# SamsungLabs/Metis

Hardware: NVIDIA H100
Metric: candidate plans evaluated/sec (higher is better)
Workload: dtype f64

## Files before the change

metis_b200/csrc/metis_blob.cuh:

```cuda
#pragma once

#include <cuda_runtime.h>
#include <stdint.h>

#include "metis_eval.cuh"

namespace metis {

struct BlobLayout {
    uint32_t total;
    uint32_t key, lc, mem, exec_full, fb, norm, derived, tmem, bwf, bwm, runt, rune, q10e;
    uint32_t rsum, rsum_bytes;
};

static inline uint32_t align16(uint32_t v) { return (v + 15u) & ~15u; }

static inline BlobLayout make_layout(const MetisProblem &p) {
    BlobLayout l;
    uint32_t o = 0;
    const uint32_t nkey = (uint32_t)p.num_types * p.num_tp * p.num_bs;
    l.key = o;       o = align16(o + nkey * 2);
    l.lc = o;        o = align16(o + (uint32_t)p.num_keys * p.lpad * 8);
    l.mem = o;       o = align16(o + (uint32_t)p.num_keys * p.lpad * 8);
    l.exec_full = o; o = align16(o + (uint32_t)p.num_keys * 8);
    l.fb = o;        o = align16(o + (uint32_t)p.num_keys * 8);
    l.norm = o;      o = align16(o + (uint32_t)p.norm_len * 8);
    l.derived = o;   o = align16(o + (uint32_t)derived_layout(p).total * 8);
    l.tmem = o;      o = align16(o + (uint32_t)p.num_types * 8);
    l.bwf = o;       o = align16(o + (uint32_t)p.num_types * 8);
    l.bwm = o;       o = align16(o + (uint32_t)p.num_types * 8);
    l.runt = o;      o = align16(o + (uint32_t)p.num_node_sequences * p.num_types);
    l.rune = o;      o = align16(o + (uint32_t)p.num_node_sequences * p.num_types * 4);
    l.q10e = o;      o = align16(o + (uint32_t)p.num_node_sequences * p.num_types * 4);
    l.total = o;
    const uint64_t n = (uint64_t)p.num_layers + 1;
    l.rsum = (o + 127u) & ~127u;
    l.rsum_bytes = (uint32_t)((uint64_t)(2 * p.num_keys + 1) * n * n * 8);
    return l;
}

__device__ __forceinline__ Tables make_tables(const MetisProblem &p, const BlobLayout &l, const uint8_t *base,
                                              const uint8_t *gblob = nullptr) {
    Tables T;
    T.p = p;
    T.rsum = gblob ? reinterpret_cast<const double *>(gblob + l.rsum) : nullptr;
    T.key_index = reinterpret_cast<const int16_t *>(base + l.key);
    T.lc = reinterpret_cast<const double *>(base + l.lc);
    T.mem = reinterpret_cast<const double *>(base + l.mem);
    T.exec_full = reinterpret_cast<const double *>(base + l.exec_full);
    T.fb_sync = reinterpret_cast<const double *>(base + l.fb);
    T.norm_lc = reinterpret_cast<const double *>(base + l.norm);
    bind_derived(T, reinterpret_cast<const double *>(base + l.derived));
    T.type_memory = reinterpret_cast<const double *>(base + l.tmem);
    T.bw_first = reinterpret_cast<const double *>(base + l.bwf);
    T.bw_min = reinterpret_cast<const double *>(base + l.bwm);
    T.run_type = base + l.runt;
    T.run_end = reinterpret_cast<const int32_t *>(base + l.rune);
    T.q10_end = reinterpret_cast<const int32_t *>(base + l.q10e);
    return T;
}

__device__ __forceinline__ int find_block(const MetisPlanSpace &sp, int64_t ordinal) {
    int lo = 0, hi = sp.num_blocks - 1;
    while (lo < hi) {
        const int mid = (lo + hi + 1) >> 1;
        if (__ldg(&sp.blocks[mid].first_ordinal) <= ordinal) lo = mid; else hi = mid - 1;
    }
    return lo;
}

__device__ __forceinline__ bool decode_plan(const MetisPlanSpace &sp, int64_t ordinal, PlanDesc &pd, int hint = -1) {
    if (ordinal < 0 || ordinal >= sp.num_plans) return false;
    int lo;
    if (hint >= 0) {
        lo = hint;
        while (lo + 1 < sp.num_blocks && __ldg(&sp.blocks[lo + 1].first_ordinal) <= ordinal) ++lo;
    } else {
        lo = find_block(sp, ordinal);
    }
    const MetisPlanBlock b = sp.blocks[lo];
    const int64_t rel = ordinal - b.first_ordinal;
    const int64_t row = rel / sp.num_div;
    const int div = (int)(rel - row * sp.num_div);
    pd.ordinal = (uint32_t)ordinal;
    pd.ns = b.ns_idx;
    pd.S = b.num_stage;
    pd.label = b.label_stage;
    pd.batches = __ldg(&sp.batches[div]);
    const int64_t off = b.rows_offset + row * b.num_stage;
    pd.row = sp.rows + off;
    pd.geo = pack_geo(off, b.num_stage, b.label_stage, b.ns_idx, div);
    return true;
}

int stage_replay_tables(const MetisProblem *problem, void *workspace, int64_t workspace_bytes, cudaStream_t stream,
                        BlobLayout &lay, const uint8_t *&blob);

}
```

metis_b200/csrc/metis_coop.cuh:

```cuda
#pragma once

#include "metis_eval.cuh"

namespace metis {

struct CoopMail {
    int m;
    int err;
    int flag;
    int aux;
    double val;
    double val2;
    int k;
    int s_top;
    int top_skip;
    int pad2;
};

struct OneLane {
    bool reverse = false;
    MB_HD int lane() const { return 0; }
    MB_HD int width() const { return 1; }
    MB_HD bool leader() const { return true; }
    MB_HD void sync() const {}
    MB_HD bool any(bool p) const { return p; }
    MB_HD unsigned ballot(bool p) const { return p ? 1u : 0u; }
    MB_HD unsigned match_any(int) const { return 1u; }
    MB_HD int first_ge_window(const double *P, int n, int i0, int lo, double t) const {
        for (int k = 0; k < 32 && i0 + k <= n; ++k)
            if (P[i0 + k] >= t) return (k > 0 || i0 <= lo) ? i0 + k : -1;
        return -1;
    }
    MB_HD int first_ge(const double *P, int n, double t) const {
        int lo = 0, hi = n + 1;
        while (lo < hi) { const int mid = (lo + hi) >> 1; if (P[mid] >= t) hi = mid; else lo = mid + 1; }
        return lo;
    }
    MB_HD int bcast_last(int v) const { return v; }
    MB_HD static void assume_shared(const void *) {}
    MB_HD void argmax_first(double &, int &) const {}
    MB_HD void argmin_first(double &, int &) const {}
    MB_HD void imax_first(int &, int &) const {}
    MB_HD void imin_first(int &, int &) const {}
    MB_HD double max_all(double v) const { return v; }
    MB_HD int incl_scan(int v) const { return v; }
    MB_HD int last_lane(int v) const { return v; }
    MB_HD void mark(int) const {}
    MB_HD void note(int) const {}
    MB_HD void gate(int, int) const {}
};

enum CoopGate { kGateRun = 0, kGateBackward = 1, kGateLeftover = 2, kGateVote = 3, kGateAdjust = 4, kGateMemory = 5,
                kGateCost = 6 };

template <class X>
MB_HD int par_index(const X &, int i, int n) { (void)n; return i; }
MB_HD int par_index(const OneLane &x, int i, int n) { return x.reverse ? n - 1 - i : i; }

#define METIS_PAR(x, var, n) \
    for (int var##_i = (x).lane(), var = par_index((x), var##_i, (n)); var##_i < (n); \
         var##_i += (x).width(), var = par_index((x), var##_i, (n)))

struct FillState {
    int k;
    int s_top;
    bool top_skip;
};

template <int MAXS, int MAXL>
MB_HD_NOINLINE FillState seq_forward(const Tables &T, int S, Scratch<MAXS, MAXL> &w) {
    const int L = T.p.num_layers;
    const double *dlay = T.dlay;
    const int N = kH * L;
    const int lim = (N - 1 - kH) > 0 ? (N - 1 - kH) : 0;
    const int last = S - 1;
    FillState st{0, -1, false};
    if (S > 1) {
        int s = 0, j = 0;
        double c = w.capa[0];
        bool done = false;
#pragma unroll 1
        for (int r = 0; r + 1 < L && !done; ++r) {
            const double d = dlay[r];
            const int nsub = (r == L - 2) ? kH - 1 : kH;
            if (nsub == kH && c > 9.0 * d) {
                c -= d; c -= d; c -= d; c -= d; c -= d; c -= d; c -= d;
                j += kH;
                continue;
            }
#pragma unroll
            for (int q = 0; q < kH; ++q) {
                if (q < nsub && !done) {
                    if (c > d) {
                        c -= d;
                    } else {
                        w.capa[s] = c;
                        w.fe[s] = (uint16_t)((j + q) | kBroke);
                        ++s;
                        if (s >= last) done = true;
                        else c = w.capa[s];
                    }
                }
            }
            j += nsub;
        }
        if (s < last) {
            w.capa[s] = c;
            w.fe[s] = (uint16_t)lim;
#pragma unroll 1
            for (int t = s + 1; t < last; ++t) w.fe[t] = (uint16_t)lim;
            st.k = lim;
            st.s_top = s;
        } else {
            st.k = (w.fe[last - 1] & kPos) + 1;
            st.s_top = last - 1;
            st.top_skip = true;
        }
    }
    return st;
}

template <int MAXS, int MAXL>
MB_HD_NOINLINE int seq_backward(const Tables &T, int S, Scratch<MAXS, MAXL> &w, int k) {
    const int L = T.p.num_layers;
    const double *dlay = T.dlay;
    const int N = kH * L;
    const int last = S - 1;
    double c = w.capa[last];
    int r = L - 1;
    double d = dlay[r];
#pragma unroll 1
    for (int i = 0; i < kH; ++i) c -= d;
    int m = N - kH;
    bool full = false;
#pragma unroll 1
    while (m > k && !full) {
        --r;
        d = dlay[r];
        const int floor_j = kH * r > k ? kH * r : k;
#pragma unroll 1
        while (m > floor_j) {
            if (!(c > d)) { full = true; break; }
            c -= d;
            --m;
        }
    }
    if (!full) {
        int sp = S - 2;
#pragma unroll 1
        while (m > 0) {
            const int j = m - 1;
#pragma unroll 1
            while (sp >= 0 && (!(w.fe[sp] & kBroke) || (int)(w.fe[sp] & kPos) > j)) --sp;
            if (!(sp >= 0 && (int)(w.fe[sp] & kPos) == j)) break;
            const double dj = dlay[j / kH];
            if (!(c > dj)) break;
            c -= dj;
            m = j;
            w.fe[sp] |= kTaken;
        }
    }
    w.capa[last] = c;
    return m;
}

template <int MAXS, int MAXL>
MB_HD_NOINLINE int seq_skipped(const Tables &T, int S, Scratch<MAXS, MAXL> &w) {
    const double *dlay = T.dlay;
    const int last = S - 1;
    int start = 0;
#pragma unroll 1
    for (int s = 0; s < last; ++s) {
        const uint16_t e = w.fe[s];
        const int pos = e & kPos;
        const int next_start = pos + ((e & kBroke) ? 1 : 0);
        if ((e & (kBroke | kTaken)) != kBroke) { start = next_start; continue; }
        const int j = pos;
        int lo = 0;
        if (pos > start) {
            lo = s;
        } else {
#pragma unroll 1
            for (int u = s;; --u) {
                if (u < s) {
                    const int t = w.lstk[u];
                    const bool above = (t == last) || (fwd_nonempty(w, t) && fwd_start(w, t) > j);
                    if (!above) { lo = t; break; }
                }
                if (fwd_nonempty(w, u)) { lo = u; break; }
                if (u == 0) break;
            }
        }
        int hi = s + 1;
        if (hi < last && !((int)(w.fe[hi] & kPos) > next_start && !w.got[hi])) {
            ++hi;
#pragma unroll 1
            while (hi < last && (!fwd_nonempty(w, hi) || w.got[hi])) ++hi;
        }
        if (lo > hi) return METIS_FATAL_SCRATCH;
        int pick = lo;
        double best = w.capa[lo];
#pragma unroll 1
        for (int t = lo + 1; t <= hi; ++t)
            if (w.capa[t] > best) { best = w.capa[t]; pick = t; }
        w.capa[pick] -= dlay[j / kH];
        w.lstk[s] = (uint8_t)pick;
        w.got[pick] = 1;
        start = next_start;
    }
    return METIS_FATAL_NONE;
}

template <int MAXS, int MAXL>
MB_HD int middle_lo(int S, const Scratch<MAXS, MAXL> &w, const FillState &st) {
    const int last = S - 1;
    if (st.s_top < 0) return 0;
#pragma unroll 1
    for (int u = st.s_top;; --u) {
        if (u < st.s_top || st.top_skip) {
            const uint16_t eu = w.fe[u];
            if ((eu & (kBroke | kTaken)) == kBroke) {
                const int t2 = w.lstk[u];
                if (t2 != last) return t2;
            }
        }
        if (fwd_nonempty(w, u)) return u;
        if (u == 0) break;
    }
    return 0;
}

MB_HD_NOINLINE double seq_py_sum(const double *v, int n) {
    if (n <= 0) return 0.0;
    double f = 0.0 + v[0], c = 0.0;
#pragma unroll 4
    for (int i = 1; i < n; ++i) {
        const double x = v[i];
        const double t = f + x;
        if (fabs(f) >= fabs(x)) c += (f - t) + x;
        else c += (x - t) + f;
        f = t;
    }
    if (c != 0.0 && isfinite(c)) f += c;
    return f;
}

template <class X>
MB_HD_NOINLINE int psub_search(const X &x, const double *P, int N, int i0, int lo, double t) {
    int i = x.first_ge_window(P, N, i0, lo, t);
    if (i < 0) {
        x.note(kPathFirstGe);
        i = x.first_ge(P, N, t);
        if (i < lo) i = lo;
    }
    return i;
}

MB_HD unsigned bucket_of(double u) {
#ifdef __CUDA_ARCH__
    return __double2uint_rz(u);
#else
    return u > 0.0 ? (unsigned)u : 0u;
#endif
}

template <class X>
MB_HD int psub_lookup(const X &x, const double *P, const uint16_t *IX, double scale, int N, int lo, double t, double &p) {
    int i = IX[bucket_of(t * scale)];
    if (i < lo) i = lo;
    const double *q = P + i;
    const double pm = q[-1], p0 = q[0], p1 = q[1];
    if ((pm < t || i == lo) && p1 >= t) {
        const bool up = !(p0 >= t);
        p = up ? p1 : p0;
        return up ? i + 1 : i;
    }
    i = psub_search(x, P, N, i, lo, t);
    p = P[i];
    return i;
}

template <int MAXS, int MAXL, class X, bool ONE = false>
struct CoopEvaluator : PlanEvaluator<MAXS, MAXL, SerialUniform, ONE> {
    using Base = PlanEvaluator<MAXS, MAXL, SerialUniform, ONE>;
    using Base::T; using Base::w; using Base::pd; using Base::bs_total; using Base::nbad; using Base::aux;
    X x;
    CoopMail &mail;

    MB_HD CoopEvaluator(const Tables &t, Scratch<MAXS, MAXL> &s, CoopMail &mb, const X &lanes)
        : Base(t, s), x(lanes), mail(mb) {}

    MB_HD void shared_scratch() const { X::assume_shared(&w); X::assume_shared(&mail); }

    MB_HD void begin_coop(const PlanDesc &plan) {
        shared_scratch();
        pd = plan;
        bs_total = T.p.gbs / pd.batches;
        int lb = 0;
#pragma unroll 1
        while ((2 << lb) <= bs_total) ++lb;
        nbad = 0;
        x.sync();
        int carry = 0;
#pragma unroll 1
        for (int base = 0; base < pd.S; base += x.width()) {
            const int s = base + x.lane();
            const int g = s < pd.S ? pd.row[s] : 0;
            const int sz = s < pd.S ? (1 << g) : 0;
            const int inc = x.incl_scan(sz);
            if (s < pd.S) {
                w.gcode[s] = (uint8_t)g;
                w.tpc[s] = (uint8_t)(g > lb ? g - lb : 0);
                w.rs[s] = (uint16_t)(carry + inc - sz);
            }
            carry += x.last_lane(inc);
        }
        if (x.leader()) w.rs[pd.S] = (uint16_t)carry;
        x.sync();
    }

    MB_HD bool next_strategy_coop(bool have_state) {
        shared_scratch();
        int pick = 0x7FFFFFFF;
        if (have_state) {
            double best = INFINITY;
            bool none = true;
            METIS_PAR(x, s, pd.S) {
                if (w.gcode[s] != w.tpc[s] && (none || w.mstate[s] < best || (w.mstate[s] == best && s < pick))) {
                    pick = s; best = w.mstate[s]; none = false;
                }
            }
            x.argmin_first(best, pick);
        } else {
            int best = -1;
            METIS_PAR(x, s, pd.S) {
                const int ldp = (int)w.gcode[s] - (int)w.tpc[s];
                if (ldp != 0 && (ldp > best || (ldp == best && s < pick))) { pick = s; best = ldp; }
            }
            x.imax_first(best, pick);
        }
        if (pick == 0x7FFFFFFF) return false;
        const int g = w.gcode[pick], t = w.tpc[pick];
        nbad += (this->stage_bad(g, t + 1) ? 1 : 0) - (this->stage_bad(g, t) ? 1 : 0);
        x.sync();
        if (x.leader()) w.tpc[pick] = (uint8_t)(t + 1);
        x.sync();
        return true;
    }

    MB_HD_NOINLINE int first_error(const double *box, int n) {
        shared_scratch();
        x.sync();
        if (x.leader()) {
            mail.err = 0;
#pragma unroll 1
            for (int s = 0; s < n; ++s)
                if (box[s] != 0.0) {
                    uint32_t a;
                    mail.err = decode_error(box[s], a);
                    mail.aux = (int)a;
                    break;
                }
        }
        x.sync();
        aux = (uint32_t)mail.aux;
        return mail.err;
    }

    MB_HD int compute_performance_coop() {
        shared_scratch();
        bool failed = false;
        x.sync();
        METIS_PAR(x, s, pd.S) {
            double p;
            const int rc = this->stage_performance(s, p);
            w.perf[s] = p;
            w.extra[s] = encode_error(rc, aux);
            failed = failed || rc != 0;
        }
        if (x.any(failed)) return first_error(w.extra, pd.S);
        x.sync();
        if (x.leader()) mail.val = seq_py_sum(w.perf, pd.S);
        x.sync();
        const double tot = mail.val;
        if (tot == 0.0) return METIS_FATAL_ZERODIV;
        METIS_PAR(x, s, pd.S) w.perf[s] = w.perf[s] / tot;
        x.sync();
        return 0;
    }

    MB_HD bool forward_coop() {
        shared_scratch();
        const int S = pd.S, last = S - 1;
        const int L = T.p.num_layers;
        if (S < 4 || T.p.norm_len < L) { x.note(kPathSeqForward); return false; }
        const int N = kH * L;
        const int lim = (N - 1 - kH) > 0 ? (N - 1 - kH) : 0;
        const double *dsub = T.dsub;
        const double *P = T.psub;
        int a = 0, first_open = -1;
        const double scale = T.pidx[0];
        if (scale > 0.0) {
            const uint16_t *IX = reinterpret_cast<const uint16_t *>(T.pidx + 1);
            const double plim = P[lim];
            double pa = P[0];
            int s = 0;
#pragma unroll 1
            for (; s < last; ++s) {
                const double t = w.perf[s] + pa;
                if (!(a < lim && t <= plim)) break;
                const int i = psub_lookup(x, P, IX, scale, N, a + 1, t, pa);
                if (x.leader()) { w.first[s] = (uint16_t)a; w.fe[s] = (uint16_t)((i - 1) | kBroke); }
                a = i;
            }
            if (s < last) {
                first_open = s;
                if (x.leader()) {
#pragma unroll 1
                    for (int u = s; u < last; ++u) { w.first[u] = (uint16_t)(u == s ? a : lim); w.fe[u] = (uint16_t)lim; }
                }
                a = lim;
            }
        } else {
            int span = lim / last;
#pragma unroll 1
            for (int s = 0; s < last; ++s) {
                int b = lim;
                bool closed = false;
                if (a < lim) {
                    const double t = w.perf[s] + P[a];
                    int i0 = a + span - 14;
                    if (i0 < a + 1) i0 = a + 1;
                    int i = x.first_ge_window(P, N, i0, a + 1, t);
                    if (i < 0) { x.note(kPathFirstGe); i = x.first_ge(P, N, t); }
                    b = i - 1 > a ? i - 1 : a;
                    if (b >= lim) b = lim; else closed = true;
                    span = b - a;
                }
                if (x.leader()) { w.first[s] = (uint16_t)a; w.fe[s] = (uint16_t)(b | (closed ? kBroke : 0)); }
                if (!closed && first_open < 0) first_open = s;
                a = closed ? b + 1 : lim;
            }
        }
        x.sync();
        x.mark(19);
        bool bad = false;
        METIS_PAR(x, s, last) {
            const int st = w.first[s];
            const uint16_t e = w.fe[s];
            const int b = e & kPos;
            double c = w.perf[s];
            bool fits = true;
#pragma unroll 4
            for (int j = st; j < b; ++j) {
                const double d = dsub[j];
                fits &= c > d;
                c -= d;
            }
            if (!fits || ((e & kBroke) && c > dsub[b])) bad = true;
            w.capa[s] = c;
        }
        if (x.any(bad)) {
            x.note(kPathVerifyFailed);
            x.sync();
            METIS_PAR(x, s, last) w.capa[s] = w.perf[s];
            return false;
        }
        if (x.leader()) {
            if (first_open < 0) { mail.k = a; mail.s_top = last - 1; mail.top_skip = 1; }
            else { mail.k = lim; mail.s_top = first_open; mail.top_skip = 0; }
        }
        return true;
    }

    MB_HD int fill_coop() {
        shared_scratch();
        const int S = pd.S, last = S - 1;
        const double *dlay = T.dlay;
        x.sync();
        const bool fwd = forward_coop();
        x.sync();
        x.gate(kGateBackward, 11);
        if (x.leader()) {
            if (!fwd) {
                x.mark(18);
                const FillState st = seq_forward<MAXS, MAXL>(T, S, w);
                mail.k = st.k; mail.s_top = st.s_top; mail.top_skip = st.top_skip ? 1 : 0;
                x.mark(11);
            }
            mail.m = seq_backward<MAXS, MAXL>(T, S, w, mail.k);
            mail.err = 0;
        }
        x.sync();
        x.gate(kGateLeftover, 12);
        const FillState st{mail.k, mail.s_top, mail.top_skip != 0};
        const int m = mail.m;
        if (st.s_top >= 0 && !st.top_skip) x.note(kPathTail);
        const int reach = st.s_top;
        bool irregular = false;
        METIS_PAR(x, s, reach + 1) {
            const int start = s == 0 ? 0 : (int)(w.fe[s - 1] & kPos) + ((w.fe[s - 1] & kBroke) ? 1 : 0);
            if (!((int)(w.fe[s] & kPos) > start)) irregular = true;
        }
        irregular = x.any(irregular);
        if (irregular) {
            x.note(kPathIrregular);
            if (x.leader()) mail.err = seq_skipped<MAXS, MAXL>(T, S, w);
            x.sync();
            if (mail.err) return mail.err;
        } else if (reach >= 0) {
            int carry = 0;
#pragma unroll 1
            for (int base = 0; base <= last; base += x.width()) {
                const int s = base + x.lane();
                bool has = false, o0 = false, o1 = false, has_prev = false;
                double c = 0.0, d = 0.0, d_prev = 0.0;
                int pos = 0;
                if (s <= last) {
                    c = w.capa[s];
                    if (s > 0 && s - 1 < last) {
                        const uint16_t ep = w.fe[s - 1];
                        has_prev = (ep & (kBroke | kTaken)) == kBroke;
                        if (has_prev) d_prev = dlay[(ep & kPos) / kH];
                    }
                    if (s < last) {
                        const uint16_t e = w.fe[s];
                        has = (e & (kBroke | kTaken)) == kBroke;
                        if (has) {
                            pos = e & kPos;
                            d = dlay[pos / kH];
                            const double cn = w.capa[s + 1];
                            o0 = cn > c;
                            o1 = has_prev ? cn > (c - d_prev) : o0;
                        }
                    }
                }
                const unsigned kmask = x.ballot(o0 == o1), vmask = x.ballot(o0);
                const unsigned below_me = x.lane() ? (0xFFFFFFFFu >> (32 - x.lane())) : 0u;
                const unsigned kin = kmask & below_me;
                const bool in = kin ? ((vmask >> (31 - clz32(kin))) & 1u) != 0u : carry != 0;
                const bool up = (o0 == o1) ? o0 : in;
                carry = x.bcast_last(up ? 1 : 0);
                x.sync();
                if (s <= last) {
                    double cc = c;
                    const bool got_prev = has_prev && in;
                    if (got_prev) cc -= d_prev;
                    if (has && !up) cc -= d;
                    if (got_prev || (has && !up)) w.capa[s] = cc;
                    if (has) w.lstk[s] = (uint8_t)(up ? s + 1 : s);
                }
            }
            x.sync();
        }
        x.mark(17);
        if (m > st.k) {
            x.note(kPathMiddle);
            if (x.leader()) mail.flag = middle_lo<MAXS, MAXL>(S, w, st);
            x.sync();
            int lo = mail.flag;
#pragma unroll 1
            for (int j = st.k; j < m; ++j) {
                int pick = 0x7FFFFFFF;
                double best = -INFINITY;
#pragma unroll 1
                for (int t = lo + x.lane(); t <= last; t += x.width())
                    if (w.capa[t] > best || (w.capa[t] == best && t < pick)) { best = w.capa[t]; pick = t; }
                x.argmax_first(best, pick);
                x.sync();
                if (x.leader()) {
                    w.capa[pick] = best - dlay[j / kH];
                    reinterpret_cast<uint8_t *>(w.subw)[j - st.k] = (uint8_t)pick;
                }
                x.sync();
                if (pick != last) lo = pick;
            }
        }
        return METIS_FATAL_NONE;
    }

    MB_HD int balance_coop() {
        shared_scratch();
        const int S = pd.S;
        const int L = T.p.num_layers;
        if (T.p.norm_len < L) return METIS_FATAL_INDEX;
        const double *lc = T.norm_lc;
        const int last = S - 1;
        x.sync();
        METIS_PAR(x, s, S) { w.capa[s] = w.perf[s]; w.got[s] = 0; }
        x.sync();
        x.mark(10);
        const int rc_tail = fill_coop();
        if (rc_tail) return rc_tail;
        const int m = mail.m;
        x.gate(kGateVote, 13);
        const int kfwd = mail.k;
        const int B = (L + 31) >> 5;
        METIS_PAR(x, blk, 32) {
            const int r0 = blk * B, r1 = r0 + B < L ? r0 + B : L;
            const int j0 = kH * r0;
            int t = 0;
            if (j0 < kfwd && j0 < m) {
                int lo = 0, hi = last - 1;
#pragma unroll 1
                while (lo < hi) {
                    const int mid = (lo + hi) >> 1;
                    const uint16_t e = w.fe[mid];
                    if ((int)(e & kPos) + ((e & kBroke) ? 1 : 0) <= j0) lo = mid + 1; else hi = mid;
                }
                t = lo;
            }
            uint16_t e = w.fe[t];
            int nxt = (int)(e & kPos) + ((e & kBroke) ? 1 : 0);
#pragma unroll 1
            for (int r = r0; r < r1; ++r) {
                int own = last;
                if (kH * r < m) {
                    uint64_t v = 0xFF00000000000000ULL;
#pragma unroll 1
                    for (int q = 0; q < kH; ++q) {
                        const int j = kH * r + q;
                        int st;
                        if (j >= m) st = last;
                        else if (j >= kfwd) st = reinterpret_cast<const uint8_t *>(w.subw)[j - kfwd];
                        else {
#pragma unroll 1
                            while (nxt <= j) { ++t; e = w.fe[t]; nxt = (int)(e & kPos) + ((e & kBroke) ? 1 : 0); }
                            st = t;
                            if (nxt - 1 == j && (e & kBroke)) st = (e & kTaken) ? last : (int)w.lstk[t];
                        }
                        v |= (uint64_t)st << (8 * q);
                    }
                    own = layer_owner(v, (T.p.corrected & METIS_FIX_Q5) != 0);
                }
                reinterpret_cast<uint8_t *>(w.ownerw)[r] = (uint8_t)own;
            }
        }
        METIS_PAR(x, s, S) w.cnt[s] = 0;
        x.sync();
        x.mark(14);
#pragma unroll 1
        for (int base = 0; base < L; base += x.width()) {
            const int r = base + x.lane();
            const int own = r < L ? (int)reinterpret_cast<const uint8_t *>(w.ownerw)[r] : (int)kDropped;
            const unsigned peers = x.match_any(own);
            if (own != (int)kDropped && x.lane() == ctz32(peers)) {
                const int n = popc32(peers), lo_r = r, hi_r = base + 31 - clz32(peers);
                const int have = w.cnt[own];
                if (have == 0 || lo_r < (int)w.first[own]) w.first[own] = (uint16_t)lo_r;
                if (have == 0 || hi_r > (int)w.lastl[own]) w.lastl[own] = (uint16_t)hi_r;
                w.cnt[own] = (uint16_t)(have + n);
            }
            x.sync();
        }
        METIS_PAR(x, s, S) {
            const int n = w.cnt[s];
            w.capa[s] = n ? w.perf[s] - range_sum<SerialUniform>(T, kRangeNorm, 0, lc, w.first[s], (int)w.lastl[s] + 1) : w.perf[s];
        }
        x.sync();
        x.gate(kGateAdjust, 15);
        uint8_t *owner = reinterpret_cast<uint8_t *>(w.ownerw);
#pragma unroll 1
        for (int n = 1; n <= 3; ++n) {
            int top = 0x7FFFFFFF;
            double maxc = -INFINITY;
            METIS_PAR(x, t, S)
                if (w.capa[t] > maxc || (w.capa[t] == maxc && t < top)) { maxc = w.capa[t]; top = t; }
            x.argmax_first(maxc, top);
            if (top == 0x7FFFFFFF) top = 0;
            int nb = -1;
            double val = INFINITY;
            if (top - 1 >= 0 && w.capa[top - 1] < val) { nb = top - 1; val = w.capa[top - 1]; }
            if (top + 1 < S && w.capa[top + 1] < val) { nb = top + 1; }
            if (nb < 0 || w.cnt[nb] <= 1) break;
            const int layer = (top > nb) ? w.lastl[nb] : w.first[nb];
            const double dl = lc[layer];
            const double ntop = w.capa[top] - dl;
            const double nnb = w.capa[nb] + dl;
            double newmax = -INFINITY;
            METIS_PAR(x, t, S) {
                const double v = (t == top) ? ntop : (t == nb) ? nnb : w.capa[t];
                if (v > newmax) newmax = v;
            }
            newmax = x.max_all(newmax);
            if (newmax > maxc) break;
            x.sync();
            if (x.leader()) {
                owner[layer] = (uint8_t)top;
                w.capa[top] = ntop;
                w.capa[nb] = nnb;
                if (top > nb) { int r = layer - 1; while (owner[r] != nb) --r; w.lastl[nb] = (uint16_t)r; }
                else          { int r = layer + 1; while (owner[r] != nb) ++r; w.first[nb] = (uint16_t)r; }
                if (w.cnt[top] == 0) { w.first[top] = (uint16_t)layer; w.lastl[top] = (uint16_t)layer; }
                else {
                    if (layer < (int)w.first[top]) w.first[top] = (uint16_t)layer;
                    if (layer > (int)w.lastl[top]) w.lastl[top] = (uint16_t)layer;
                }
                ++w.cnt[top];
                --w.cnt[nb];
            }
            x.sync();
        }
        x.mark(16);
        int carry = 0;
#pragma unroll 1
        for (int base = 0; base < S; base += x.width()) {
            const int s = base + x.lane();
            const int v = s < S ? (int)w.cnt[s] : 0;
            const int inc = x.incl_scan(v);
            if (s < S) w.part[s + 1] = (uint16_t)(carry + inc);
            carry += x.last_lane(inc);
        }
        if (x.leader()) w.part[0] = 0;
        x.sync();
        return METIS_FATAL_NONE;
    }

    MB_HD int adjust_performance_coop() {
        shared_scratch();
        const int S = pd.S;
        double *ratio = reinterpret_cast<double *>(w.subw);
        x.sync();
        METIS_PAR(x, s, S) {
            double av, adj, extra;
            this->stage_adjust(s, av, adj, extra);
            w.capa[s] = av;
            w.mstate[s] = adj;
            ratio[s] = extra;
        }
        x.sync();
        if (x.leader()) {
            double need = 0.;
#pragma unroll 4
            for (int s = 0; s < S; ++s) need += ratio[s];
            mail.val = need;
            mail.flag = seq_py_sum(w.capa, S) < need ? 1 : 0;
        }
        x.sync();
        if (mail.flag) return 1;
        METIS_PAR(x, s, S) w.extra[s] = 0.;
        x.sync();
        if (x.leader()) {
            double need = mail.val;
            int guard = 0;
            mail.err = 0;
#pragma unroll 1
            while (need > 0.01) {
                PySum tot;
#pragma unroll 4
                for (int s = 0; s < S; ++s) tot.add(w.capa[s] > 0.001 ? w.perf[s] : 0.0);
                const double tmp_total = tot.result();
#pragma unroll 4
                for (int s = 0; s < S; ++s)
                    ratio[s] = w.capa[s] > 0.001 ? w.perf[s] / tmp_total : 0.0;
#pragma unroll 4
                for (int s = 0; s < S; ++s) {
                    const double av = w.capa[s];
                    const double want = need * ratio[s];
                    const double give = want > av ? av : want;
                    w.extra[s] += give;
                    w.capa[s] -= give;
                    need -= give;
                }
                if (++guard > 4096) { mail.err = METIS_FATAL_HANG; break; }
            }
        }
        x.sync();
        if (mail.err) return -mail.err;
        METIS_PAR(x, s, S) w.perf[s] = w.extra[s] + w.mstate[s];
        x.sync();
        return 0;
    }

    template <class Sink>
    MB_HD int memory_phase_coop(int attempt, Sink &sink, bool report) {
        shared_scratch();
        const int S = pd.S;
        bool failed = false, oom = false;
        x.sync();
        METIS_PAR(x, s, S) {
            double md, state;
            const int rc = this->stage_memory(s, md, state);
            w.extra[s] = md;
            w.capa[s] = state;
            w.mstate[s] = encode_error(rc, aux);
            failed = failed || rc != 0;
            oom = oom || state < 0;
        }
        failed = x.any(failed);
        oom = x.any(oom);
        if (failed) return -first_error(w.mstate, S);
        x.sync();
        if (!oom) {
            METIS_PAR(x, s, S) w.mstate[s] = w.capa[s];
            x.sync();
            return 1;
        }
        if constexpr (SinkMisses<Sink>::value) {
            if (report) {
                double m = INFINITY;
                int at = 0x7FFFFFFF;
                METIS_PAR(x, s, S)
                    if (w.capa[s] < m || (w.capa[s] == m && s < at)) { m = w.capa[s]; at = s; }
                x.argmin_first(m, at);
                sink.miss(pd, attempt, -m, at);
            }
        } else {
            (void)sink, (void)report;
        }
        if (attempt >= 3) return 0;
        x.mark(21);
        const int rc = adjust_performance_coop();
        if (rc < 0) return rc;
        return rc == 1 ? 0 : 2;
    }

    MB_HD int get_cost_coop(double &cost_out) {
        shared_scratch();
        const bool one_type = ONE || T.p.num_types == 1;
        const int nstage = pd.label < pd.S ? pd.label : pd.S;
        if (T.p.q10_devices < T.p.total_devices && this->rank_start(nstage) > T.p.q10_devices) return 1;
        double *ppterm = reinterpret_cast<double *>(w.subw);
        bool bad = false;
        double max_len = -INFINITY, max_upd = -INFINITY, max_dp = -INFINITY;
        x.sync();
        METIS_PAR(x, s, nstage) {
            double len, dpc, upd;
            if (this->stage_time(s, len)) bad = true;
            w.capa[s] = len;
            if (len > max_len) max_len = len;
            this->stage_terms(s, nstage, ppterm[s], dpc, upd);
            if (dpc > max_dp) max_dp = dpc;
            if (upd > max_upd) max_upd = upd;
        }
        if (x.any(bad)) return 1;
        max_len = x.max_all(max_len);
        max_upd = x.max_all(max_upd);
        max_dp = x.max_all(max_dp);
        x.sync();
        x.mark(23);
        if (x.leader()) {
            double pp_cost = 0.;
#pragma unroll 4
            for (int s = 0; s + 1 < nstage; ++s) pp_cost += ppterm[s];
            const double lens = seq_py_sum(w.capa, nstage);
            const int s = nstage - 1;
            const int a = one_type ? 0 : this->rank_start(s), b = a + this->group(s);
            double v = 0.0;
            mail.flag = this->fb_sync_cost(a, b, w.tpc[s], bs_total >> (w.gcode[s] - w.tpc[s]), v);
            const double fb_sync = v * (double)pd.batches;
            const double exec = ((double)(pd.batches - 1) * max_len) + lens;
            const double bg = T.p.batch_generator * (double)pd.batches;
            mail.val = exec + fb_sync + max_upd + max_dp + pp_cost + bg;
        }
        x.sync();
        if (mail.flag) return 1;
        cost_out = mail.val;
        return 0;
    }

    enum Start { kFresh = 0, kReplay = 1, kRetry = 2, kAdvance = 3 };
    template <class Sink>
    MB_HD void run_chain(const PlanDesc &plan, Sink &sink, int start, const double *perf = nullptr, size_t perf_stride = 0) {
        begin_coop(plan);
        bool started = false, have_state = false;
        bool skip_first = start == kReplay;
        int nrep = 0, step = 0;
        int call = start == kAdvance ? 1 : 0;
        if (start == kRetry) {
            METIS_PAR(x, s, pd.S) w.perf[s] = perf[(size_t)s * perf_stride];
            x.sync();
        }
#pragma unroll 1
        for (;;) {
            if (nrep == 1) return;
            int attempt = 0;
#pragma unroll 1
            for (;;) {
                int first_attempt = 1;
                if (!started) {
                    started = true;
                    if (start == kAdvance && !next_strategy_coop(false)) return;
                    if (start == kRetry) first_attempt = 2;
                } else if (!next_strategy_coop(have_state)) return;
                if (!this->valid()) continue;
                miss_call(sink, call++);
                int rc = 0;
                if (first_attempt == 1) {
                    if (!skip_first) sink.partition_call();
                    x.mark(2);
                    rc = compute_performance_coop();
                    if (rc) { sink.fatal(pd.ordinal, rc, aux); return; }
                }
                attempt = 0;
#pragma unroll 1
                for (int a = first_attempt; a <= 3; ++a) {
                    const bool fresh = !skip_first;
                    if (fresh) sink.balancer_run();
                    skip_first = false;
                    x.gate(kGateRun, 9);
                    rc = balance_coop();
                    if (rc) { sink.fatal(pd.ordinal, rc, aux); return; }
                    x.gate(kGateMemory, 20);
                    const int r = memory_phase_coop(a, sink, fresh);
                    if (r < 0) { sink.fatal(pd.ordinal, -r, aux); return; }
                    if (r == 1) { attempt = a; break; }
                    if (r == 0) break;
                }
                skip_first = false;
                have_state = attempt > 0;
                if (attempt > 0) break;
            }
            nrep = attempt;
            x.gate(kGateCost, 22);
            double cost = 0.0;
            if (get_cost_coop(cost) == 0) sink.emit(pd, step, nrep, cost, w.tpc, w.part);
            else sink.keyerror();
            x.sync();
            x.mark(24);
            ++step;
        }
    }
};

}
```

metis_b200/csrc/metis_eval.cuh:

```cuda
#pragma once

#include <stdint.h>
#include <string.h>
#include <math.h>

#include "../../include/metis_b200.h"

#if defined(__CUDACC__)
#define MB_HD __host__ __device__ __forceinline__
#define MB_HD_NOINLINE __host__ __device__ __noinline__ inline
#else
#define MB_HD inline
#define MB_HD_NOINLINE inline
#endif

namespace metis {

constexpr int kH = 7;
constexpr double kMemCoef = 5.0;
constexpr uint8_t kDropped = 0xFF;

struct Tables {
    MetisProblem p;
    const int16_t *key_index;
    const double *lc;
    const double *mem;
    const double *exec_full;
    const double *fb_sync;
    const double *norm_lc;
    const double *type_memory, *bw_first, *bw_min;
    const uint8_t *run_type;
    const int32_t *run_end;
    const int32_t *q10_end;
    const double *dlay;
    const double *inv_exec;
    const double *ratio;
    const double *dpk;
    const double *pp_hidden;
    const double *pp_vocab;
    const double *psub;
    const double *dsub;
    const double *pidx;
    const double *rsum;
};

constexpr int kDpk = 16;

struct DerivedLayout {
    int dlay, inv_exec, ratio, dpk, pp_hidden, pp_vocab, psub, dsub, pidx, total;
};

MB_HD DerivedLayout derived_layout(const MetisProblem &p) {
    DerivedLayout d;
    int o = 0;
    d.dlay = o; o += p.norm_len;
    d.inv_exec = o; o += p.num_keys;
    d.ratio = o; o += p.num_layers + 1;
    d.dpk = o; o += kDpk;
    d.pp_hidden = o; o += p.num_bs + 1;
    d.pp_vocab = o; o += (p.num_bs + 1) * p.num_tp;
    d.psub = o; o += (p.norm_len >= p.num_layers) ? kH * p.num_layers + 1 : 0;
    d.dsub = o; o += (p.norm_len >= p.num_layers) ? kH * p.num_layers : 0;
    d.pidx = o; o += (p.norm_len >= p.num_layers) ? 1 + (kH * p.num_layers + 1 + 3) / 4 : 0;
    d.total = o;
    return d;
}

MB_HD double psub_at(double acc, double lc_r, int q) { return acc + lc_r * ((double)q / 7.0); }

MB_HD double psub_index_entry(const MetisProblem &p, const double *norm_lc, int k) {
    const int L = p.num_layers, N = kH * L;
    const int lim = (N - 1 - kH) > 0 ? (N - 1 - kH) : 0;
    bool ok = N > 0;
    double acc = 0.0;
    for (int r = 0; r < L; ++r) {
        ok = ok && norm_lc[r] >= 0.0 && norm_lc[r] <= 1.7976931348623157e308;
        acc += norm_lc[r];
    }
    const double top = L < p.norm_len ? psub_at(acc, norm_lc[L], 0) : acc;
    const double scale = ok && top > 0.0 && top <= 1.7976931348623157e308 ? (double)N / top : 0.0;
    if (!(scale > 0.0 && scale <= 1.7976931348623157e308)) return 0.0;
    if (k == 0) return scale;
    double f[kH];
    for (int q = 0; q < kH; ++q) f[q] = (double)q / 7.0;
    uint64_t bits = 0;
    int r = 0;
    acc = 0.0;
    for (int e = 0; e < 4; ++e) {
        const double g = (double)(4 * (k - 1) + e);
        int ix = lim;
        while (kH * r < lim) {
            const double nxt = acc + norm_lc[r];
            if (nxt * scale >= g) {
                int q = 0;
                while (q < kH && !((acc + norm_lc[r] * f[q]) * scale >= g)) ++q;
                ix = kH * r + q < lim ? kH * r + q : lim;
                break;
            }
            acc = nxt;
            ++r;
        }
        bits |= (uint64_t)ix << (16 * e);
    }
    double v;
    memcpy(&v, &bits, sizeof(v));
    return v;
}

MB_HD double derive_entry(const MetisProblem &p, const DerivedLayout &d, const double *norm_lc,
                          const double *exec_full, const double *bw_first, int i) {
    if (i < d.inv_exec) return norm_lc[i - d.dlay] / 7.0;
    if (i < d.ratio) return 1. / exec_full[i - d.inv_exec];
    if (i < d.dpk) return (double)(i - d.ratio) / (double)p.num_layers;
    const double bw = bw_first[0] * 1048576.0;
    if (i < d.pp_hidden) {
        const int dp = 1 << (i - d.dpk);
        return (double)(2 * (dp - 1)) / ((double)dp * bw);
    }
    if (i < d.pp_vocab) return (double)((int64_t)(i - d.pp_hidden) * p.sequence_length * p.hidden_size) / bw;
    if (i >= d.pidx) return psub_index_entry(p, norm_lc, i - d.pidx);
    if (i >= d.dsub) return norm_lc[(i - d.dsub) / kH] / 7.0;
    if (i >= d.psub) {
        const int j = i - d.psub, r = j / kH;
        double acc = 0.0;
        for (int t = 0; t < r; ++t) acc += norm_lc[t];
        return r < p.norm_len ? psub_at(acc, norm_lc[r], j - r * kH) : acc;
    }
    const int e = i - d.pp_vocab;
    const int mbs = e / p.num_tp, tpc = e - mbs * p.num_tp;
    return ((double)((int64_t)mbs * p.sequence_length * p.vocab_size) / (double)(1 << tpc)) / bw;
}

MB_HD void bind_derived(Tables &T, const double *base) {
    const DerivedLayout d = derived_layout(T.p);
    T.dlay = base + d.dlay;
    T.inv_exec = base + d.inv_exec;
    T.ratio = base + d.ratio;
    T.dpk = base + d.dpk;
    T.pp_hidden = base + d.pp_hidden;
    T.pp_vocab = base + d.pp_vocab;
    T.psub = base + d.psub;
    T.dsub = base + d.dsub;
    T.pidx = base + d.pidx;
}

struct PlanDesc {
    uint32_t ordinal;
    int ns;
    int S;
    int label;
    int batches;
    const uint8_t *row;
    uint64_t geo;
};

MB_HD uint64_t pack_geo(int64_t row_offset, int S, int label, int ns, int div) {
    return (uint64_t)(row_offset & 0xFFFFFFFFLL) | ((uint64_t)((S - 1) & 0xFF) << 32) | ((uint64_t)((label - 1) & 0xFF) << 40) |
           ((uint64_t)(ns & 0xFF) << 48) | ((uint64_t)(div & 0xFF) << 56);
}

enum BalancerPath {
    kPathVerifyFailed = 0,
    kPathSeqForward = 1,
    kPathIrregular = 2,
    kPathMiddle = 3,
    kPathFirstGe = 4,
    kPathTail = 5,
    kPathVoteEnds = 6,
};

struct Serial {
    static constexpr bool kUniform = false;
    MB_HD void mark(int) const {}
    MB_HD void note(int) const {}
    MB_HD void converge() const {}
    MB_HD void rejoin(bool) {}
};
#if defined(__CUDACC__) && defined(METIS_PROFILE_PHASES)
constexpr int kBulkBatches = 31;
__device__ long long g_bulk_acc[32];
__shared__ long long s_bulk_t[32];
__shared__ int s_bulk_cur[32];
__device__ __forceinline__ void bulk_mark(unsigned group, int id) {
    __syncwarp(group);
    if ((int)(threadIdx.x & 31) == __ffs((int)group) - 1) {
        const int wi = threadIdx.x >> 5;
        const long long now = clock64();
        if (id == 1) atomicAdd((unsigned long long *)&g_bulk_acc[kBulkBatches], 1ULL);
        else atomicAdd((unsigned long long *)&g_bulk_acc[s_bulk_cur[wi] & 31], (unsigned long long)(now - s_bulk_t[wi]));
        s_bulk_cur[wi] = id;
        s_bulk_t[wi] = now;
    }
    __syncwarp(group);
}
#endif
#if defined(__CUDACC__)
struct Lockstep : Serial {
    unsigned mask;
    __device__ Lockstep() : mask(0xFFFFFFFFu) {}
    __device__ void converge() const { __syncwarp(mask); }
    __device__ void rejoin(bool p) { mask = __ballot_sync(0xFFFFFFFFu, p); }
#if defined(METIS_PROFILE_PHASES)
    __device__ void mark(int id) const { bulk_mark(__activemask(), id); }
#endif
};
#endif
struct SerialUniform : Serial {
    static constexpr bool kUniform = true;
};

constexpr uint64_t kOnes = 0x0101010101010101ULL;

constexpr uint16_t kBroke = 0x8000;
constexpr uint16_t kTaken = 0x4000;
constexpr uint16_t kPos = 0x3FFF;

template <int MAXS, int MAXL>
struct Scratch {
    double perf[MAXS];
    double capa[MAXS];
    double mstate[MAXS];
    double extra[MAXS];
    uint16_t fe[MAXS];
    uint16_t first[MAXS], lastl[MAXS], cnt[MAXS];
    uint16_t part[MAXS + 1];
    uint16_t rs[MAXS + 1];
    uint8_t gcode[MAXS];
    uint8_t tpc[MAXS];
    uint8_t lstk[MAXS];
    uint8_t got[MAXS];
    uint64_t ownerw[MAXL / 8 + 1];
    uint64_t subw[MAXL];
    static_assert(MAXL >= MAXS, "after the vote, subw holds one double per stage (CoopEvaluator's adjust and cost)");
};

MB_HD double py_sum_range(const double *x, int a, int b) {
    if (a >= b) return 0.0;
    double f = 0.0 + x[a];
    double c = 0.0;
    for (int i = a + 1; i < b; ++i) {
        const double v = x[i];
        const double t = f + v;
        if (fabs(f) >= fabs(v)) c += (f - t) + v;
        else c += (v - t) + f;
        f = t;
    }
    if (c != 0.0 && isfinite(c)) f += c;
    return f;
}

MB_HD_NOINLINE double py_sum_range_compact(const double *x, int a, int b) {
    if (a >= b) return 0.0;
    double f = 0.0 + x[a];
    double c = 0.0;
#pragma unroll 1
    for (int i = a + 1; i < b; ++i) {
        const double v = x[i];
        const double t = f + v;
        if (fabs(f) >= fabs(v)) c += (f - t) + v;
        else c += (v - t) + f;
        f = t;
    }
    if (c != 0.0 && isfinite(c)) f += c;
    return f;
}

template <class X>
MB_HD double sum_range(const double *x, int a, int b) {
    if constexpr (X::kUniform) return py_sum_range_compact(x, a, b);
    else return py_sum_range(x, a, b);
}

MB_HD void fill_range_sums(const double *row, int L, int a, double *out) {
    const int n = L + 1;
    double f = 0.0 + row[a];
    double c = 0.0;
    out[(size_t)(a + 1) * n + a] = f;
#if defined(__CUDA_ARCH__)
#pragma unroll 1
#endif
    for (int i = a + 1; i < L; ++i) {
        const double v = row[i];
        const double t = f + v;
        if (fabs(f) >= fabs(v)) c += (f - t) + v;
        else c += (v - t) + f;
        f = t;
        out[(size_t)(i + 1) * n + a] = (c != 0.0 && isfinite(c)) ? f + c : f;
    }
}
MB_HD int range_sum_tables(const MetisProblem &p) { return 2 * p.num_keys + 1; }
MB_HD const double *range_sum_row(const MetisProblem &p, int t, const double *mem, const double *lc, const double *norm) {
    if (t < p.num_keys) return mem + (size_t)t * p.lpad;
    if (t < 2 * p.num_keys) return lc + (size_t)(t - p.num_keys) * p.lpad;
    return p.norm_len >= p.num_layers ? norm : nullptr;
}

enum RangeTable { kRangeMem = 0, kRangeLc = 1, kRangeNorm = 2 };
template <class X>
MB_HD double range_sum(const Tables &T, int family, int key, const double *row, int a, int b) {
    if (a >= b) return 0.0;
    if (T.rsum && b <= T.p.num_layers) {
        const int n = T.p.num_layers + 1;
        const int t = family == kRangeMem ? key : family == kRangeLc ? T.p.num_keys + key : 2 * T.p.num_keys;
#if defined(__CUDA_ARCH__)
        return __ldg(&T.rsum[((size_t)t * n + b) * n + a]);
#else
        return T.rsum[((size_t)t * n + b) * n + a];
#endif
    }
    return sum_range<X>(row, a, b);
}

struct PySum {
    double f, c;
    int n;
    MB_HD PySum() : f(0.0), c(0.0), n(0) {}
    MB_HD void add(double v) {
        if (n == 0) { f = 0.0 + v; }
        else {
            const double t = f + v;
            if (fabs(f) >= fabs(v)) c += (f - t) + v;
            else c += (v - t) + f;
            f = t;
        }
        ++n;
    }
    MB_HD double result() const {
        double r = f;
        if (c != 0.0 && isfinite(c)) r += c;
        return r;
    }
};

MB_HD double pow2_neg(int k) {
    const uint64_t bits = (uint64_t)(1023 - k) << 52;
    double d;
    memcpy(&d, &bits, sizeof(d));
    return d;
}

MB_HD int type_of_rank(const Tables &T, int ns, int rank) {
    const int nt = T.p.num_types;
    const int32_t *end = T.run_end + ns * nt;
    const uint8_t *typ = T.run_type + ns * nt;
#pragma unroll 1
    for (int k = 0; k < nt; ++k)
        if (rank < end[k]) return typ[k];
    return typ[nt - 1];
}

MB_HD int type_of_q10(const Tables &T, int ns, int idx) {
    const int nt = T.p.num_types;
    const int32_t *end = T.q10_end + ns * nt;
    const uint8_t *typ = T.run_type + ns * nt;
#pragma unroll 1
    for (int k = 0; k < nt; ++k)
        if (idx < end[k]) return typ[k];
    return typ[nt - 1];
}

MB_HD int key_of(const Tables &T, int type, int tpc, int bs) {
    if (tpc >= T.p.num_tp || bs < 1 || bs > T.p.num_bs) return -1;
    return T.key_index[(type * T.p.num_tp + tpc) * T.p.num_bs + (bs - 1)];
}

template <int MAXS, int MAXL>
MB_HD int fwd_start(const Scratch<MAXS, MAXL> &w, int s) {
    if (s == 0) return 0;
    const uint16_t e = w.fe[s - 1];
    return (e & kPos) + ((e & kBroke) ? 1 : 0);
}

template <int MAXS, int MAXL>
MB_HD bool fwd_nonempty(const Scratch<MAXS, MAXL> &w, int s) {
    return (int)(w.fe[s] & kPos) > fwd_start(w, s);
}

MB_HD int popc64(uint64_t v) {
#if defined(__CUDA_ARCH__)
    return __popcll(v);
#else
    return __builtin_popcountll(v);
#endif
}
MB_HD int ctz64(uint64_t v) {
#if defined(__CUDA_ARCH__)
    return __ffsll((long long)v) - 1;
#else
    return __builtin_ctzll(v);
#endif
}
MB_HD int popc32(uint32_t v) {
#if defined(__CUDA_ARCH__)
    return __popc(v);
#else
    return __builtin_popcount(v);
#endif
}
MB_HD int ctz32(uint32_t v) {
#if defined(__CUDA_ARCH__)
    return __ffs((int)v) - 1;
#else
    return __builtin_ctz(v);
#endif
}
MB_HD int clz32(uint32_t v) {
#if defined(__CUDA_ARCH__)
    return __clz((int)v);
#else
    return __builtin_clz(v);
#endif
}
MB_HD int clz64(uint64_t v) {
#if defined(__CUDA_ARCH__)
    return __clzll((long long)v);
#else
    return __builtin_clzll(v);
#endif
}

MB_HD uint64_t swar_eq(uint64_t x, int c) {
    const uint64_t y = x ^ ((uint64_t)c * kOnes);
    const uint64_t lo7 = 0x7F7F7F7F7F7F7F7FULL;
    return ~((((y & lo7) + lo7) | y) | lo7);
}

MB_HD int swar_count(uint64_t x, int c) { return popc64(swar_eq(x, c) & 0x0080808080808080ULL); }

MB_HD int layer_owner(uint64_t v, bool plurality) {
    if (plurality) {
        int best = 0, own = (int)kDropped;
#pragma unroll 1
        for (int q = 0; q < kH; ++q) {
            const int cq = (int)((v >> (8 * q)) & 0xFF);
            const int n = swar_count(v, cq);
            if (n > best || (n == best && cq < own)) { best = n; own = cq; }
        }
        return own;
    }
    const int c3 = (int)((v >> 24) & 0xFF);
    if (swar_count(v, c3) * 2 > kH) return c3;
    const int c0 = (int)(v & 0xFF), c1 = (int)((v >> 8) & 0xFF), c2 = (int)((v >> 16) & 0xFF);
    if (swar_count(v, c0) * 2 > kH) return c0;
    if (c1 != c0 && swar_count(v, c1) * 2 > kH) return c1;
    if (c2 != c1 && c2 != c0 && swar_count(v, c2) * 2 > kH) return c2;
    return (int)kDropped;
}

template <int MAXS, int MAXL, class X>
MB_HD int balance_run(const Tables &T, int S, Scratch<MAXS, MAXL> &w, const X &x) {
    const int L = T.p.num_layers;
    if (T.p.norm_len < L) return METIS_FATAL_INDEX;
    const double *dlay = T.dlay;
    const double *lc = T.norm_lc;
    const int N = kH * L;
    const int lim = (N - 1 - kH) > 0 ? (N - 1 - kH) : 0;
    const int last = S - 1;
    int broken = METIS_FATAL_NONE;

#pragma unroll (X::kUniform ? 1 : 0)
    for (int s = 0; s < S; ++s) { w.got[s] = 0; w.cnt[s] = 0; }

    x.mark(10);
    int k = 0, sTop = -1;
    bool topSkip = false;
    if (S > 1) {
        int s = 0, j = 0;
        double c = w.perf[0];
#pragma unroll (X::kUniform ? 1 : 0)
        for (int r = 0; r + 1 < L; ++r) {
            const double d = dlay[r];
            const int nsub = (r == L - 2) ? kH - 1 : kH;
#pragma unroll
            for (int q = 0; q < kH; ++q) {
                if (q < nsub) {
                    if (s < last) {
                        if (c > d) {
                            c -= d;
                        } else {
                            w.capa[s] = c;
                            w.fe[s] = (uint16_t)(j | kBroke);
                            ++s;
                            c = w.perf[s];
                        }
                    }
                    ++j;
                }
            }
        }
        if (s < last) {
            x.note(kPathTail);
            w.capa[s] = c;
            w.fe[s] = (uint16_t)lim;
#pragma unroll (X::kUniform ? 1 : 0)
            for (int t = s + 1; t < last; ++t) { w.capa[t] = w.perf[t]; w.fe[t] = (uint16_t)lim; }
            k = lim;
            sTop = s;
        } else {
            k = (w.fe[last - 1] & kPos) + 1;
            sTop = last - 1;
            topSkip = true;
        }
    }

    x.mark(11);
    x.converge();
    int m;
    {
        double c = w.perf[last];
        const double dl = dlay[L - 1];
#pragma unroll (X::kUniform ? 1 : 0)
        for (int i = 0; i < kH; ++i) c -= dl;
        m = N - kH;
        int sp = S - 2;
#pragma unroll (X::kUniform ? 1 : 0)
        while (m > 0) {
            const int j = m - 1;
            bool un = (j >= k);
            if (!un) {
#pragma unroll (X::kUniform ? 1 : 0)
                while (sp >= 0 && (!(w.fe[sp] & kBroke) || (int)(w.fe[sp] & kPos) > j)) --sp;
                un = (sp >= 0 && (int)(w.fe[sp] & kPos) == j);
            }
            if (!un) break;
            const double d = dlay[j / kH];
            if (!(c > d)) break;
            c -= d;
            m = j;
            if (j < k) w.fe[sp] |= kTaken;
        }
        w.capa[last] = c;
    }

    x.mark(12);
    x.converge();
    {
        int start = 0;
#pragma unroll (X::kUniform ? 1 : 0)
        for (int s = 0; s < last; ++s) {
            const uint16_t e = w.fe[s];
            const int pos = e & kPos;
            const int next_start = pos + ((e & kBroke) ? 1 : 0);
            if ((e & (kBroke | kTaken)) != kBroke) { start = next_start; continue; }
            const int j = pos;
            int lo = 0;
            if (pos > start) {
                lo = s;
            } else {
                x.note(kPathIrregular);
#pragma unroll (X::kUniform ? 1 : 0)
                for (int u = s;; --u) {
                    if (u < s) {
                        const int t = w.lstk[u];
                        const bool above = (t == last) || (fwd_nonempty(w, t) && fwd_start(w, t) > j);
                        if (!above) { lo = t; break; }
                    }
                    if (fwd_nonempty(w, u)) { lo = u; break; }
                    if (u == 0) break;
                }
            }
            int hi = s + 1;
            if (hi < last && !((int)(w.fe[hi] & kPos) > next_start && !w.got[hi])) {
                ++hi;
#pragma unroll (X::kUniform ? 1 : 0)
                while (hi < last && (!fwd_nonempty(w, hi) || w.got[hi])) ++hi;
            }
            if (lo > hi) { broken = METIS_FATAL_SCRATCH; hi = lo; }
            int pick = lo;
            double best = w.capa[lo];
#pragma unroll (X::kUniform ? 1 : 0)
            for (int t = lo + 1; t <= hi; ++t)
                if (w.capa[t] > best) { best = w.capa[t]; pick = t; }
            w.capa[pick] -= dlay[j / kH];
            w.lstk[s] = (uint8_t)pick;
            w.got[pick] = 1;
            start = next_start;
        }
    }
    x.converge();
    const int nblk = m - k;
    if (nblk > 0) x.note(kPathMiddle);
    uint8_t *mid = reinterpret_cast<uint8_t *>(w.subw);
    {
        int below = -1;
#pragma unroll (X::kUniform ? 1 : 0)
        for (int t = 0; t < nblk; ++t) {
            const int j = k + t;
            int lo = 0;
            if (below >= 0) lo = below;
            else if (sTop >= 0) {
#pragma unroll (X::kUniform ? 1 : 0)
                for (int u = sTop;; --u) {
                    if (u < sTop || topSkip) {
                        const uint16_t eu = w.fe[u];
                        if ((eu & (kBroke | kTaken)) == kBroke) {
                            const int t2 = w.lstk[u];
                            if (t2 != last) { lo = t2; break; }
                        }
                    }
                    if (fwd_nonempty(w, u)) { lo = u; break; }
                    if (u == 0) break;
                }
            }
            int pick = lo;
            double best = w.capa[lo];
#pragma unroll (X::kUniform ? 1 : 0)
            for (int t2 = lo + 1; t2 <= last; ++t2)
                if (w.capa[t2] > best) { best = w.capa[t2]; pick = t2; }
            w.capa[pick] -= dlay[j / kH];
            if (pick != last) below = pick;
            mid[t] = (uint8_t)pick;
        }
    }

    x.mark(13);
    x.converge();
    if (k > 0) x.note(kPathVoteEnds);
    int t = 0, nxt = 0;
    uint16_t e = 0;
    if (k > 0) { e = w.fe[0]; nxt = (int)(e & kPos) + ((e & kBroke) ? 1 : 0); }
    const bool plurality = (T.p.corrected & METIS_FIX_Q5) != 0;
    int run_own = (int)kDropped, run_first = 0, run_len = 0;
#pragma unroll (X::kUniform ? 1 : 0)
    for (int r = 0; r < L; ++r) {
        int own = last;
        if (kH * r < m) {
            uint64_t v = 0xFF00000000000000ULL;
#pragma unroll
            for (int q = 0; q < kH; ++q) {
                const int j = kH * r + q;
                int st = last;
                if (j < k) {
#pragma unroll 1
                    while (nxt <= j) { ++t; e = w.fe[t]; nxt = (int)(e & kPos) + ((e & kBroke) ? 1 : 0); }
                    st = t;
                    if (nxt - 1 == j && (e & kBroke)) st = (e & kTaken) ? last : (int)w.lstk[t];
                } else if (j < m) {
                    st = mid[j - k];
                }
                v |= (uint64_t)(uint32_t)st << (8 * q);
            }
            own = layer_owner(v, plurality);
        }
        reinterpret_cast<uint8_t *>(w.ownerw)[r] = (uint8_t)own;
        {
            if (own == run_own) ++run_len;
            else {
                if (run_own != (int)kDropped) {
                    if (w.cnt[run_own] == 0) w.first[run_own] = (uint16_t)run_first;
                    w.lastl[run_own] = (uint16_t)(r - 1);
                    w.cnt[run_own] = (uint16_t)(w.cnt[run_own] + run_len);
                }
                run_own = own; run_first = r; run_len = 1;
            }
        }
    }
    if (run_own != (int)kDropped) {
        if (w.cnt[run_own] == 0) w.first[run_own] = (uint16_t)run_first;
        w.lastl[run_own] = (uint16_t)(L - 1);
        w.cnt[run_own] = (uint16_t)(w.cnt[run_own] + run_len);
    }
    x.mark(14);
    x.converge();
    uint8_t *owner = reinterpret_cast<uint8_t *>(w.ownerw);
    int top = 0x7FFFFFFF;
    double maxc = -INFINITY;
#pragma unroll (X::kUniform ? 1 : 0)
    for (int s = 0; s < S; ++s) {
        const double c = w.cnt[s] ? w.perf[s] - range_sum<X>(T, kRangeNorm, 0, lc, w.first[s], (int)w.lastl[s] + 1) : w.perf[s];
        w.capa[s] = c;
        if (c > maxc) { maxc = c; top = s; }
    }

    x.mark(15);
    x.converge();
#pragma unroll (X::kUniform ? 1 : 0)
    for (int n = 1; n <= 3; ++n) {
        if (top == 0x7FFFFFFF) top = 0;
        int nb = -1;
        double val = INFINITY;
        if (top - 1 >= 0 && w.capa[top - 1] < val) { nb = top - 1; val = w.capa[top - 1]; }
        if (top + 1 < S && w.capa[top + 1] < val) { nb = top + 1; }
        if (nb < 0 || w.cnt[nb] <= 1) break;
        const int layer = (top > nb) ? w.lastl[nb] : w.first[nb];
        const double dl = lc[layer];
        const double ntop = w.capa[top] - dl;
        const double nnb = w.capa[nb] + dl;
        double newmax = -INFINITY;
        int newtop = 0x7FFFFFFF;
#pragma unroll (X::kUniform ? 1 : 0)
        for (int t = 0; t < S; ++t) {
            const double v = (t == top) ? ntop : (t == nb) ? nnb : w.capa[t];
            if (v > newmax) { newmax = v; newtop = t; }
        }
        if (newmax > maxc) break;
        owner[layer] = (uint8_t)top;
        w.capa[top] = ntop;
        w.capa[nb] = nnb;
        if (top > nb) { int r = layer - 1; while (owner[r] != nb) --r; w.lastl[nb] = (uint16_t)r; }
        else          { int r = layer + 1; while (owner[r] != nb) ++r; w.first[nb] = (uint16_t)r; }
        if (w.cnt[top] == 0) { w.first[top] = (uint16_t)layer; w.lastl[top] = (uint16_t)layer; }
        else {
            if (layer < (int)w.first[top]) w.first[top] = (uint16_t)layer;
            if (layer > (int)w.lastl[top]) w.lastl[top] = (uint16_t)layer;
        }
        ++w.cnt[top];
        --w.cnt[nb];
        maxc = newmax;
        top = newtop;
    }

    x.mark(16);
    x.converge();
    w.part[0] = 0;
#pragma unroll (X::kUniform ? 1 : 0)
    for (int s = 0; s < S; ++s) w.part[s + 1] = (uint16_t)(w.part[s] + w.cnt[s]);
    return broken;
}

struct HSplit {
    int nruns;
    int type[METIS_MAX_TYPES];
    int n[METIS_MAX_TYPES];
    int base[METIS_MAX_TYPES];
    int plus[METIS_MAX_TYPES];
};

MB_HD_NOINLINE int partition_data(const Tables &T, int ns, int rank_lo, int count, int dp, int tpc, int bs,
                                  HSplit &out, uint32_t &aux, bool q10 = false) {
    const int gsz = count / dp;
    double perf[METIS_MAX_TYPES];
    PySum total;
    out.nruns = 0;
#pragma unroll 1
    for (int i = 0; i < dp; ++i) {
        const int t = q10 ? type_of_q10(T, ns, rank_lo + i * gsz) : type_of_rank(T, ns, rank_lo + i * gsz);
        if (out.nruns == 0 || out.type[out.nruns - 1] != t) {
            const int key = key_of(T, t, tpc, 1);
            if (key < 0) { aux = ((uint32_t)tpc << 16) | 1u; return METIS_FATAL_KEY_EXEC; }
            const double e = T.exec_full[key];
            if (e == 0.0) return METIS_FATAL_ZERODIV;
            out.type[out.nruns] = t;
            out.n[out.nruns] = 0;
            perf[out.nruns] = 1. / e;
            ++out.nruns;
        }
        ++out.n[out.nruns - 1];
        total.add(perf[out.nruns - 1]);
    }
    const double tot = total.result();
    double frac[METIS_MAX_TYPES];
    int assigned = 0;
#pragma unroll 1
    for (int r = 0; r < out.nruns; ++r) {
        const double v = (double)bs * (perf[r] / tot);
        const int b = (int)v;
        out.base[r] = b;
        out.plus[r] = 0;
        frac[r] = v - (double)b;
        assigned += b * out.n[r];
    }
    int rem = bs - assigned;
    bool used[METIS_MAX_TYPES];
#pragma unroll 1
    for (int r = 0; r < out.nruns; ++r) used[r] = false;
#pragma unroll 1
    for (int it = 0; it < out.nruns && rem > 0; ++it) {
        int pick = -1;
#pragma unroll 1
        for (int r = 0; r < out.nruns; ++r)
            if (!used[r] && (pick < 0 || frac[r] > frac[pick])) pick = r;
        used[pick] = true;
        const int g = rem < out.n[pick] ? rem : out.n[pick];
        out.plus[pick] = g;
        rem -= g;
    }
    if (rem > 0) return METIS_FATAL_SCRATCH;
    return METIS_FATAL_NONE;
}

template <class Sink, class = void>
struct SinkMisses { static constexpr bool value = false; };
template <class Sink>
struct SinkMisses<Sink, decltype(void(Sink::kMisses))> { static constexpr bool value = Sink::kMisses; };
template <class Sink>
MB_HD void miss_call(Sink &sink, int call) {
    if constexpr (SinkMisses<Sink>::value) sink.call = call;
    else (void)sink, (void)call;
}

struct TraceTap {
    double *demand;
    double *state;
    double cost[5];
};

MB_HD int halvings_of(const MetisProblem &p, int S, const uint8_t *gcode, const uint8_t *tpc, int bs_total) {
    int ltp = 0, lbs = 0;
    while ((2 << ltp) <= p.max_tp) ++ltp;
    while ((2 << lbs) <= p.max_bs) ++lbs;
    int u = 0;
#if defined(__CUDA_ARCH__)
#pragma unroll 1
#endif
    for (int s = 0; s < S; ++s) {
        const int g = gcode[s], t = tpc[s];
        int lm = 0;
        while ((2 << lm) <= (bs_total >> (g - t))) ++lm;
        int room = g - t;
        if (ltp - t < room) room = ltp - t;
        if (lbs - lm < room) room = lbs - lm;
        if (room > 0) u += room;
    }
    return u;
}

MB_HD double encode_error(int rc, uint32_t aux) { return rc ? (double)rc + (double)aux * 256.0 : 0.0; }
MB_HD int decode_error(double word, uint32_t &aux) {
    const uint64_t code = (uint64_t)word;
    aux = (uint32_t)(code >> 8);
    return (int)(code & 0xFF);
}

template <int MAXS, int MAXL, class X = Serial, bool ONE = false>
struct PlanEvaluator {
    const Tables &T;
    Scratch<MAXS, MAXL> &w;
    X x;
    PlanDesc pd;
    int bs_total;
    int nbad;
    uint32_t aux;
    TraceTap *tap;

    MB_HD PlanEvaluator(const Tables &t, Scratch<MAXS, MAXL> &s, const X &lanes = X())
        : T(t), w(s), x(lanes), bs_total(0), nbad(0), aux(0), tap(nullptr) {}

    MB_HD int group(int s) const { return 1 << w.gcode[s]; }
    MB_HD int dp_of(int s) const { return (1 << w.gcode[s]) >> w.tpc[s]; }

    MB_HD bool stage_bad(int g, int t) const {
        const int mbs = bs_total >> (g - t);
        return mbs == 0 || mbs > T.p.max_bs || (1 << t) > T.p.max_tp;
    }

    MB_HD int begin(const PlanDesc &plan) {
        pd = plan;
        if (pd.S > MAXS || T.p.num_layers > MAXL) return -1;
        bs_total = T.p.gbs / pd.batches;
        int lb = 0;
#pragma unroll (X::kUniform ? 1 : 0)
        while ((2 << lb) <= bs_total) ++lb;
        nbad = 0;
        int a = 0;
        for (int s = 0; s < pd.S; ++s) {
            const int g = pd.row[s];
            const int t = g > lb ? g - lb : 0;
            if (stage_bad(g, t)) { nbad = 1; return 0; }
            w.gcode[s] = (uint8_t)g;
            w.rs[s] = (uint16_t)a;
            a += 1 << g;
            w.tpc[s] = (uint8_t)t;
        }
        w.rs[pd.S] = (uint16_t)a;
        return nbad == 0 ? 1 : 0;
    }

    MB_HD bool next_strategy(bool have_state) {
        int pick = -1;
        if (have_state) {
            double best = 0.0;
#pragma unroll (X::kUniform ? 1 : 0)
            for (int s = 0; s < pd.S; ++s)
                if (w.gcode[s] != w.tpc[s] && (pick < 0 || w.mstate[s] < best)) { pick = s; best = w.mstate[s]; }
        } else {
            int best = -1;
#pragma unroll (X::kUniform ? 1 : 0)
            for (int s = 0; s < pd.S; ++s) {
                const int ldp = (int)w.gcode[s] - (int)w.tpc[s];
                if (ldp != 0 && ldp > best) { pick = s; best = ldp; }
            }
        }
        if (pick < 0) return false;
        const int g = w.gcode[pick], t = w.tpc[pick];
        nbad += (stage_bad(g, t + 1) ? 1 : 0) - (stage_bad(g, t) ? 1 : 0);
        w.tpc[pick] = (uint8_t)(t + 1);
        return true;
    }

    MB_HD bool valid() const { return nbad == 0; }

    MB_HD int halvings() const { return halvings_of(T.p, pd.S, w.gcode, w.tpc, bs_total); }

    MB_HD double memory_capacity(int a, int b) const {
        const int nt = T.p.num_types;
        if (ONE || nt == 1) return T.type_memory[0] * (double)(b - a);
        const int32_t *end = T.run_end + pd.ns * nt;
        const uint8_t *typ = T.run_type + pd.ns * nt;
        PySum acc;
        int lo = 0;
#pragma unroll (X::kUniform ? 1 : 0)
        for (int k = 0; k < nt; ++k) {
            const int hi = end[k];
            const int x = (a > lo ? a : lo), y = (b < hi ? b : hi);
            if (y > x) acc.add(T.type_memory[typ[k]] * (double)(y - x));
            lo = hi;
        }
        return acc.result();
    }

    MB_HD int replica_perf_cost(int type, int tpc, int h, double &out) {
        double acc = 0.;
#pragma unroll (X::kUniform ? 1 : 0)
        for (int bit = 30; bit >= 0; --bit) {
            const int piece = 1 << bit;
            if (!(h & piece)) continue;
            const int key = key_of(T, type, tpc, piece);
            if (key < 0) { aux = ((uint32_t)tpc << 16) | (uint32_t)piece; return METIS_FATAL_KEY_EXEC; }
            acc += T.exec_full[key];
        }
        out = acc;
        return 0;
    }

    MB_HD_NOINLINE int hetero_performance(int a, int b, int dp, int tpc, double &p) {
        HSplit hs;
        int rc = partition_data(T, pd.ns, a, b - a, dp, tpc, bs_total, hs, aux);
        if (rc) return rc;
        double mx = -INFINITY;
#pragma unroll (X::kUniform ? 1 : 0)
        for (int r = 0; r < hs.nruns; ++r) {
            double c;
            if (hs.plus[r] > 0) {
                rc = replica_perf_cost(hs.type[r], tpc, hs.base[r] + 1, c);
                if (rc) return rc;
                if (c > mx) mx = c;
            }
            if (hs.plus[r] < hs.n[r]) {
                rc = replica_perf_cost(hs.type[r], tpc, hs.base[r], c);
                if (rc) return rc;
                if (c > mx) mx = c;
            }
        }
        p = (mx != 0.0) ? 1. / mx : 0.0;
        return 0;
    }

    MB_HD int rank_start(int s) const { return w.rs[s]; }


    MB_HD int stage_performance(int s, double &p) {
        const int g = w.gcode[s], tpc = w.tpc[s];
        const int a = rank_start(s), b = a + (1 << g);
        int ta = 0, tb = 0;
        if (!(ONE || T.p.num_types == 1)) { ta = type_of_rank(T, pd.ns, a); tb = type_of_rank(T, pd.ns, b - 1); }
        p = 0.0;
        if (ta != tb) return hetero_performance(a, b, 1 << (g - tpc), tpc, p);
        const int bs = bs_total >> (g - tpc);
        const int key = key_of(T, ta, tpc, bs);
        if (key < 0) { aux = ((uint32_t)tpc << 16) | (uint32_t)bs; return METIS_FATAL_KEY_EXEC; }
        if (T.exec_full[key] == 0.0) return METIS_FATAL_ZERODIV;
        p = T.inv_exec[key];
        return 0;
    }

    MB_HD int stage_memory(int s, double &demand, double &state) {
        const bool one_type = ONE || T.p.num_types == 1;
        const bool own_type = (T.p.corrected & METIS_FIX_Q6) != 0;
        const int g = w.gcode[s], tpc = w.tpc[s];
        const int a = rank_start(s), b = a + (1 << g);
        int rc = 0;
        demand = 0.001;
        if (!ONE && own_type) {
            rc = memory_demand_own_type(s, demand);
        } else if (T.p.q10_devices < T.p.total_devices && !own_type && b > T.p.q10_devices) {
            aux = 0;
            rc = METIS_FATAL_INDEX;
        } else if (one_type || type_of_q10(T, pd.ns, a) == type_of_q10(T, pd.ns, b - 1)) {
            const int bs = bs_total >> (g - tpc);
            const int key = key_of(T, T.run_type[pd.ns * T.p.num_types], tpc, bs);
            if (key < 0) { aux = ((uint32_t)tpc << 16) | (uint32_t)bs; rc = METIS_FATAL_KEY_MEMORY; }
            else demand += range_sum<X>(T, kRangeMem, key, T.mem + (size_t)key * T.p.lpad, w.part[s], w.part[s + 1]) * kMemCoef;
        } else {
            rc = hetero_memory_demand(s, T.run_type[pd.ns * T.p.num_types], demand);
        }
        state = memory_capacity(a, b) - demand;
        return rc;
    }

    MB_HD void stage_adjust(int s, double &avail, double &adj, double &extra) const {
        const double c = w.perf[s], md = w.extra[s];
        const double mc = memory_capacity(rank_start(s), rank_start(s) + group(s));
        if (mc > md) {
            adj = c;
            avail = (c * mc / md) - c;
            extra = 0.0;
        } else {
            avail = 0.0;
            adj = c * (mc / md) * 0.9;
            extra = c - adj;
        }
    }

    MB_HD bool stage_time(int s, double &len) {
        const bool one_type = ONE || T.p.num_types == 1;
        const int g = w.gcode[s], tpc = w.tpc[s];
        const int a = one_type ? 0 : rank_start(s), b = a + (1 << g);
        const int la = w.part[s], lb = w.part[s + 1];
        const int ldp = g - tpc;
        const int ta = one_type ? 0 : type_of_rank(T, pd.ns, a);
        const int tb = one_type ? 0 : type_of_rank(T, pd.ns, b - 1);
        len = 0.0;
        if (ta != tb) return hetero_exec_cost(a, b, 1 << ldp, tpc, la, lb, len) != 0;
        const int key = key_of(T, ta, tpc, bs_total >> ldp);
        if (key < 0) return true;
        len = range_sum<X>(T, kRangeLc, key, T.lc + (size_t)key * T.p.lpad, la, lb);
        return false;
    }

    MB_HD void stage_terms(int s, int nstage, double &pp, double &dpc, double &upd) const {
        const int per = T.p.devices_per_node;
        const int Lm = T.p.num_layers;
        const bool ubw = T.p.uniform_bw != 0;
        const int g = w.gcode[s], tpc = w.tpc[s];
        const int la = w.part[s], lb = w.part[s + 1];
        const int ldp = g - tpc;
        const int mbs = bs_total >> ldp;
        const double inv_tp = pow2_neg(tpc);
        pp = 0.0;
        if (s < nstage - 1) {
            if (ubw) {
                pp = (lb == Lm - 1) ? T.pp_vocab[mbs * T.p.num_tp + tpc] : T.pp_hidden[mbs];
            } else {
                double act;
                if (lb == Lm - 1)
                    act = (double)((int64_t)mbs * T.p.sequence_length * T.p.vocab_size) * inv_tp;
                else
                    act = (double)((int64_t)mbs * T.p.sequence_length * T.p.hidden_size);
                pp = act / (bw_of_node_range(rank_start(s) / per, (rank_start(s + 2) - 1) / per) * 1048576.0);
            }
        }
        int ntr = lb - la;
        double params = 0.0;
        if (la == 0) { params += T.p.input_params * inv_tp; --ntr; }
        if (lb == Lm) { params += T.p.output_params * inv_tp; --ntr; }
        params += T.p.transformer_params * inv_tp * (double)ntr;
        if (ubw) dpc = T.dpk[ldp] * params;
        else {
            const int dp = 1 << ldp;
            dpc = (double)(2 * (dp - 1)) / ((double)dp * (dp_bandwidth(rank_start(s), dp, 1 << tpc) * 1048576.0)) * params;
        }
        upd = T.p.optimizer_time * inv_tp * T.ratio[lb - la];
    }


    MB_HD int compute_performance() {
        PySum total;
        int rc = 0;
#pragma unroll (X::kUniform ? 1 : 0)
        for (int s = 0; s < pd.S; ++s) {
            double p;
            rc = stage_performance(s, p);
            if (rc) break;
            w.perf[s] = p;
            total.add(p);
        }
        x.converge();
        if (rc) return rc;
        const double tot = total.result();
        if (tot == 0.0) return METIS_FATAL_ZERODIV;
#pragma unroll (X::kUniform ? 1 : 0)
        for (int s = 0; s < pd.S; ++s) w.perf[s] = w.perf[s] / tot;
        return 0;
    }

    MB_HD_NOINLINE int hetero_memory_demand(int s, int type0, double &demand) {
        const int la = w.part[s], lb = w.part[s + 1], tpc = w.tpc[s];
        HSplit hs;
        const int rc = partition_data(T, pd.ns, 0, T.p.q10_devices, dp_of(s), tpc, bs_total, hs, aux, true);
        if (rc) return rc;
#pragma unroll (X::kUniform ? 1 : 0)
        for (int r = 0; r < hs.nruns; ++r)
#pragma unroll (X::kUniform ? 1 : 0)
            for (int i = 0; i < hs.n[r]; ++i) {
                const int h = hs.base[r] + (i < hs.plus[r] ? 1 : 0);
#pragma unroll (X::kUniform ? 1 : 0)
                for (int bit = 30; bit >= 0; --bit) {
                    const int piece = 1 << bit;
                    if (!(h & piece)) continue;
                    const int key = key_of(T, type0, tpc, piece);
                    if (key < 0) { aux = ((uint32_t)tpc << 16) | (uint32_t)piece; return METIS_FATAL_KEY_MEMORY; }
                    demand += range_sum<X>(T, kRangeMem, key, T.mem + (size_t)key * T.p.lpad, la, lb) * kMemCoef;
                }
            }
        return 0;
    }

    MB_HD_NOINLINE int memory_demand_own_type(int s, double &demand) {
        const int la = w.part[s], lb = w.part[s + 1], tpc = w.tpc[s], g = w.gcode[s];
        const int a = rank_start(s), b = a + (1 << g);
        const int ta = type_of_rank(T, pd.ns, a), tb = type_of_rank(T, pd.ns, b - 1);
        if (ta == tb) {
            const int bs = bs_total >> (g - tpc);
            const int key = key_of(T, ta, tpc, bs);
            if (key < 0) { aux = ((uint32_t)tpc << 16) | (uint32_t)bs; return METIS_FATAL_KEY_MEMORY; }
            demand += range_sum<SerialUniform>(T, kRangeMem, key, T.mem + (size_t)key * T.p.lpad, la, lb) * kMemCoef;
            return 0;
        }
        HSplit hs;
        const int rc = partition_data(T, pd.ns, a, b - a, 1 << (g - tpc), tpc, bs_total, hs, aux);
        if (rc) return rc;
        double worst = 0.0;
#pragma unroll 1
        for (int r = 0; r < hs.nruns; ++r)
#pragma unroll 1
            for (int v = 0; v < 2; ++v) {
                const int cntv = v ? hs.plus[r] : hs.n[r] - hs.plus[r];
                const int h = hs.base[r] + v;
                if (cntv <= 0 || h == 0) continue;
                double need = 0.0;
#pragma unroll 1
                for (int bit = 30; bit >= 0; --bit) {
                    const int piece = 1 << bit;
                    if (!(h & piece)) continue;
                    const int key = key_of(T, hs.type[r], tpc, piece);
                    if (key < 0) { aux = ((uint32_t)tpc << 16) | (uint32_t)piece; return METIS_FATAL_KEY_MEMORY; }
                    need += range_sum<SerialUniform>(T, kRangeMem, key, T.mem + (size_t)key * T.p.lpad, la, lb) * kMemCoef;
                }
                if (need > worst) worst = need;
            }
        demand += worst;
        return 0;
    }

    MB_HD_NOINLINE int adjust_performance() {
        const int S = pd.S;
        double need = 0.;
        PySum avail_sum;
#pragma unroll (X::kUniform ? 1 : 0)
        for (int s = 0; s < S; ++s) {
            double av, adj, extra;
            stage_adjust(s, av, adj, extra);
            w.capa[s] = av;
            w.mstate[s] = adj;
            w.extra[s] = 0.;
            need += extra;
            avail_sum.add(av);
        }
        if (avail_sum.result() < need) return 1;
        int guard = 0;
#pragma unroll (X::kUniform ? 1 : 0)
        while (need > 0.01) {
            PySum tot;
#pragma unroll (X::kUniform ? 1 : 0)
            for (int s = 0; s < S; ++s) tot.add(w.capa[s] > 0.001 ? w.perf[s] : 0.0);
            const double tmp_total = tot.result();
#pragma unroll (X::kUniform ? 1 : 0)
            for (int s = 0; s < S; ++s) {
                const double av = w.capa[s];
                const double ratio = av > 0.001 ? w.perf[s] / tmp_total : 0.0;
                const double want = need * ratio;
                const double give = want > av ? av : want;
                w.extra[s] += give;
                w.capa[s] -= give;
                need -= give;
            }
            if (++guard > 4096) return -METIS_FATAL_HANG;
        }
#pragma unroll (X::kUniform ? 1 : 0)
        for (int s = 0; s < S; ++s) w.perf[s] = w.extra[s] + w.mstate[s];
        return 0;
    }

    struct NoMisses {};
    MB_HD int memory_phase(int attempt) {
        NoMisses none;
        return memory_phase(attempt, none);
    }
    template <class Sink>
    MB_HD int memory_phase(int attempt, Sink &sink) {
        const int S = pd.S;
        bool oom = false;
        int rc = 0;
#pragma unroll (X::kUniform ? 1 : 0)
        for (int s = 0; s < S; ++s) {
            double md, state;
            rc = stage_memory(s, md, state);
            if (rc) break;
            w.extra[s] = md;
            w.mstate[s] = state;
            if (state < 0) oom = true;
            if (tap) { tap->demand[s] = md; tap->state[s] = state; }
        }
        x.converge();
        if (rc) return -rc;
        if (!oom) return 1;
        if constexpr (SinkMisses<Sink>::value) {
            double m = w.mstate[0];
            int at = 0;
#pragma unroll 1
            for (int s = 1; s < S; ++s)
                if (w.mstate[s] < m) { m = w.mstate[s]; at = s; }
            sink.miss(pd, attempt, -m, at);
        } else {
            (void)sink;
        }
        if (attempt >= 3) return 0;
        x.mark(21);
        const int adj = adjust_performance();
        if (adj < 0) return adj;
        return adj == 1 ? 0 : 2;
    }

    template <class Sink>
    MB_HD_NOINLINE int partition_layer(Sink &sink) {
#pragma unroll (X::kUniform ? 1 : 0)
        for (int attempt = 1; attempt <= 3; ++attempt) {
            sink.balancer_run();
            const int rc = balance_run<MAXS, MAXL>(T, pd.S, w, x);
            if (rc) return -rc;
            const int r = memory_phase(attempt, sink);
            if (r == 1) return attempt;
            if (r <= 0) return r;
        }
        return 0;
    }

    MB_HD double bw_of_node_range(int n0, int n1) const {
        const int per = T.p.devices_per_node;
        if (n0 == n1) return T.bw_first[type_of_q10(T, pd.ns, n0 * per)];
        double slow = INFINITY;
        const int nt = T.p.num_types;
        const int32_t *end = T.q10_end + pd.ns * nt;
        const uint8_t *typ = T.run_type + pd.ns * nt;
        int lo = 0;
#pragma unroll (X::kUniform ? 1 : 0)
        for (int k = 0; k < nt; ++k) {
            const int hi = end[k];
            if (hi > lo && n0 * per < hi && (n1 + 1) * per > lo) {
                const double v = T.bw_min[typ[k]];
                if (v < slow) slow = v;
            }
            lo = hi;
        }
        return slow;
    }

    MB_HD double dp_bandwidth(int a, int dp, int tp) const {
        const int per = T.p.devices_per_node;
        double slow = INFINITY;
#pragma unroll (X::kUniform ? 1 : 0)
        for (int d = 0; d < dp; ++d) {
            const int n0 = (a + d) / per;
            int nlast = n0;
            bool multi = false;
            double gmin = INFINITY;
            int tprev = -1;
#pragma unroll (X::kUniform ? 1 : 0)
            for (int i = 0; i < tp; ++i) {
                const int node = (a + d + i * dp) / per;
                if (node != nlast) { multi = true; nlast = node; }
                const int t = type_of_q10(T, pd.ns, node * per);
                if (t != tprev) { const double v = T.bw_min[t]; if (v < gmin) gmin = v; tprev = t; }
            }
            const double bw = multi ? gmin : T.bw_first[type_of_q10(T, pd.ns, n0 * per)];
            if (bw < slow) slow = bw;
        }
        return slow;
    }

    MB_HD_NOINLINE int hetero_exec_cost(int a, int b, int dp, int tpc, int la, int lb, double &len) {
        HSplit hs;
        uint32_t dummy;
        if (partition_data(T, pd.ns, a, b - a, dp, tpc, bs_total, hs, dummy)) return 1;
        len = -INFINITY;
#pragma unroll (X::kUniform ? 1 : 0)
        for (int r = 0; r < hs.nruns; ++r)
#pragma unroll (X::kUniform ? 1 : 0)
            for (int v = 0; v < 2; ++v) {
                const int cntv = v ? hs.plus[r] : hs.n[r] - hs.plus[r];
                const int h = hs.base[r] + v;
                if (cntv <= 0 || h == 0) continue;
                double acc = 0.;
#pragma unroll (X::kUniform ? 1 : 0)
                for (int bit = 30; bit >= 0; --bit) {
                    const int piece = 1 << bit;
                    if (!(h & piece)) continue;
                    if (piece > T.p.max_bs) return 1;
                    const int key = key_of(T, hs.type[r], tpc, piece);
                    if (key < 0) return 1;
                    acc += range_sum<X>(T, kRangeLc, key, T.lc + (size_t)key * T.p.lpad, la, lb);
                }
                if (acc > len) len = acc;
            }
        return 0;
    }

    MB_HD int fb_sync_cost(int a, int b, int tpc, int mbs, double &out) const {
        const int nt = T.p.num_types;
        const int32_t *end = T.run_end + pd.ns * nt;
        const uint8_t *typ = T.run_type + pd.ns * nt;
        double mx = -INFINITY;
        int lo = 0;
#pragma unroll (X::kUniform ? 1 : 0)
        for (int k = 0; k < nt; ++k) {
            const int hi = end[k];
            if ((a > lo ? a : lo) < (b < hi ? b : hi)) {
                const int key = key_of(T, typ[k], tpc, mbs);
                if (key < 0) return 1;
                const double v = T.fb_sync[key];
                if (v == 0.0) return 1;
                if (v > mx) mx = v;
            }
            lo = hi;
        }
        out = mx;
        return 0;
    }

    MB_HD int get_cost(double &cost_out) {
        const bool one_type = ONE || T.p.num_types == 1;
        const int nstage = pd.label < pd.S ? pd.label : pd.S;
        if (T.p.q10_devices < T.p.total_devices && rank_start(nstage) > T.p.q10_devices) return 1;
        bool bad = false;
        PySum lens_sum;
        double max_len = -INFINITY;
#pragma unroll (X::kUniform ? 1 : 0)
        for (int s = 0; s < nstage; ++s) {
            double len;
            if (stage_time(s, len)) bad = true;
            lens_sum.add(len);
            if (len > max_len) max_len = len;
        }
        if (bad) return 1;
        double max_upd = -INFINITY, max_dp = -INFINITY;
        double pp_cost = 0., fb_sync = 0.;
#pragma unroll (X::kUniform ? 1 : 0)
        for (int s = 0; s < nstage; ++s) {
            double pp, dpc, upd;
            stage_terms(s, nstage, pp, dpc, upd);
            if (s < nstage - 1) pp_cost += pp;
            if (dpc > max_dp) max_dp = dpc;
            if (upd > max_upd) max_upd = upd;
        }
        {
            const int s = nstage - 1;
            const int a = one_type ? 0 : rank_start(s), b = a + group(s);
            double v;
            if (fb_sync_cost(a, b, w.tpc[s], bs_total >> (w.gcode[s] - w.tpc[s]), v)) return 1;
            fb_sync = v * (double)pd.batches;
        }
        const double exec = ((double)(pd.batches - 1) * max_len) + lens_sum.result();
        const double bg = T.p.batch_generator * (double)pd.batches;
        cost_out = exec + fb_sync + max_upd + max_dp + pp_cost + bg;
        if (tap) { tap->cost[0] = exec; tap->cost[1] = fb_sync; tap->cost[2] = max_upd; tap->cost[3] = max_dp; tap->cost[4] = pp_cost; }
        return 0;
    }

    template <class Sink>
    MB_HD_NOINLINE void run(const PlanDesc &plan, Sink &sink, int only_step = -1) {
        const int ok = begin(plan);
        if (ok < 0) { sink.fatal(plan.ordinal, METIS_FATAL_SCRATCH, 0); return; }
        if (ok == 0) return;
        bool started = false, have_state = false;
        int nrep = 0, step = 0, call = 0;
#pragma unroll (X::kUniform ? 1 : 0)
        for (;;) {
            if (nrep == 1) return;
            int attempt = 0;
#pragma unroll (X::kUniform ? 1 : 0)
            for (;;) {
                if (!started) started = true;
                else if (!next_strategy(have_state)) return;
                if (!valid()) continue;
                miss_call(sink, call++);
                sink.partition_call();
                int rc = compute_performance();
                if (rc) { sink.fatal(pd.ordinal, rc, aux); return; }
                attempt = partition_layer(sink);
                if (attempt < 0) { sink.fatal(pd.ordinal, -attempt, aux); return; }
                have_state = attempt > 0;
                if (attempt > 0) break;
            }
            nrep = attempt;
            double cost;
            if (get_cost(cost) == 0) sink.emit(pd, step, nrep, cost, w.tpc, w.part);
            else sink.keyerror();
            if (only_step >= 0 && step == only_step) return;
            ++step;
        }
    }
};

template <int MAXS, int MAXL, bool ONE, class X = Serial, class Sink>
MB_HD bool first_task(const Tables &T, Scratch<MAXS, MAXL> &w, Sink &sink, bool has, const PlanDesc &plan, int &chain_hint,
                      int &resume) {
    PlanEvaluator<MAXS, MAXL, X, ONE> ev(T, w);
    bool cont = false;
    sink.phase(1);
    if (has) {
        const int ok = ev.begin(plan);
        if (ok < 0) sink.fatal(plan.ordinal, METIS_FATAL_SCRATCH, 0);
        has = ok == 1;
    }
    ev.x.rejoin(has);
    if (has) {
        miss_call(sink, 0);
        sink.partition_call();
        const int rc = ev.compute_performance();
        if (rc) { sink.fatal(plan.ordinal, rc, ev.aux); has = false; }
    }
    sink.phase(2);
    ev.x.rejoin(has);
    if (has) {
        sink.balancer_run();
        const int rc = balance_run<MAXS, MAXL>(T, plan.S, w, ev.x);
        if (rc) { sink.fatal(plan.ordinal, rc, ev.aux); has = false; }
    }
    sink.phase(3);
    ev.x.rejoin(has);
    bool costing = false;
    if (has) {
        const int r = ev.memory_phase(1, sink);
        if (r < 0) sink.fatal(plan.ordinal, -r, ev.aux);
        else if (r != 1) {
            cont = true;
            chain_hint = ev.halvings();
            resume = r == 2 ? 2 : 3;
        } else costing = true;
    }
    sink.phase(4);
    ev.x.rejoin(costing);
    if (costing) {
        double cost;
        if (ev.get_cost(cost) == 0) sink.emit(plan, 0, 1, cost, w.tpc, w.part);
        else sink.keyerror();
    }
    sink.phase(0);
    ev.x.rejoin(true);
    return cont;
}

MB_HD int homo_cost(const Tables &T, int type, int dp, int pp, int tp, int mbs, int gbs, double &cost_out,
                    int &oom, TraceTap *tap = nullptr) {
    const int L = T.p.num_layers;
    const int per = T.p.devices_per_node;
    int tpc = 0;
#pragma unroll 1
    while ((1 << tpc) < tp) ++tpc;
    const int key = ((1 << tpc) == tp) ? key_of(T, type, tpc, mbs) : -1;
    if (key < 0) return 1;
    const int num_mbs = gbs / mbs / dp;
    (void)type;
    const double intra = T.p.node0_bandwidth;
    const double inter = T.p.node0_bandwidth;
    const int base = (L - 2) / pp, rem = (L - 2) % pp;
    PySum lens_sum;
    double max_len = -INFINITY, max_params = -INFINITY, max_mem = -INFINITY;
    double pp_cost = 0., fb_sync = 0.;
    int a = 0;
#pragma unroll 1
    for (int s = 0; s < pp; ++s) {
        int count = base + ((s >= 1 && s <= rem) ? 1 : 0) + (s == 0 ? 1 : 0) + (s == pp - 1 ? 1 : 0);
        const int b = a + count;
        const double len = py_sum_range(T.lc + (size_t)key * T.p.lpad, a, b);
        lens_sum.add(len);
        if (len > max_len) max_len = len;
        PySum ps;
#pragma unroll 1
        for (int r = a; r < b && r < L; ++r) {
            const double v = (r == 0) ? T.p.input_params / (double)tp
                           : (r == L - 1) ? T.p.output_params / (double)tp
                           : T.p.transformer_params / (double)tp;
            ps.add(v);
        }
        const double sp = ps.result();
        if (sp > max_params) max_params = sp;
        const double sm = py_sum_range(T.mem + (size_t)key * T.p.lpad, a, b);
        if (sm > max_mem) max_mem = sm;
        if (tap) tap->demand[s] = sm;
        if (s == pp - 1) {
            const double v = T.fb_sync[key];
            if (v == 0.0) return 1;
            fb_sync = v * (double)num_mbs;
        } else {
            double act;
            if (b == L - 1) act = (double)((int64_t)mbs * T.p.sequence_length * T.p.vocab_size) / (double)tp;
            else act = (double)((int64_t)mbs * T.p.sequence_length * T.p.hidden_size);
            double bw = intra;
#pragma unroll 1
            for (int d = 0; d < dp; ++d)
#pragma unroll 1
                for (int t = 0; t < tp; ++t) {
                    const int r0 = s * dp * tp + d * tp + t, r1 = r0 + dp * tp;
                    if (r0 / per != r1 / per) bw = inter;
                }
            pp_cost += act / (bw * 1048576.0);
        }
        a = b;
    }
    oom = (T.p.node0_memory < max_mem) ? 1 : 0;
    const double exec = ((double)(num_mbs - 1) * max_len) + lens_sum.result();
    const double upd = T.p.optimizer_time / (double)pp / (double)tp;
    double bw = intra;
#pragma unroll 1
    for (int p = 0; p < pp; ++p)
        if ((p * dp * tp) / per != ((p + 1) * dp * tp - 1) / per) bw = inter;
    const double dpc = (double)(2 * (dp - 1)) / ((double)dp * (bw * 1048576.0)) * max_params;
    const double bg = T.p.batch_generator * (double)num_mbs;
    cost_out = exec + fb_sync + upd + dpc + pp_cost + bg;
    if (tap) { tap->cost[0] = exec; tap->cost[1] = fb_sync; tap->cost[2] = upd; tap->cost[3] = dpc; tap->cost[4] = pp_cost; }
    return 0;
}

}
```

metis_b200/csrc/metis_search.cu:

```cuda
#include <cuda_runtime.h>
#include <cooperative_groups.h>
#include <stdint.h>
#include <stdio.h>
#include <stdlib.h>
#include <string.h>

#include <type_traits>

#include "metis_eval.cuh"
#include "metis_blob.cuh"
#include "metis_coop.cuh"
#include "metis_warp.cuh"
#include "metis_trace.cuh"
#include "metis_rows.cuh"

namespace cg = cooperative_groups;

namespace metis {

#ifndef METIS_THREADS
#define METIS_THREADS 256
#endif
#ifndef METIS_MIN_BLOCKS
#define METIS_MIN_BLOCKS 3
#endif
#ifndef METIS_MIN_BLOCKS_BIG
#define METIS_MIN_BLOCKS_BIG METIS_MIN_BLOCKS
#endif
#ifndef METIS_MIN_BLOCKS_BIG_ONE
#define METIS_MIN_BLOCKS_BIG_ONE (METIS_MIN_BLOCKS + 1)
#endif
constexpr int kThreads = METIS_THREADS;
constexpr int kMaxS = METIS_MAX_STAGES;
constexpr int kMaxL = METIS_MAX_LAYERS;
constexpr int kSmemBlobMax = 160 * 1024;

static thread_local char g_err[256] = "";
static thread_local cudaEvent_t g_ev_before = nullptr, g_ev_after = nullptr;

static int cuda_fail(cudaError_t e, const char *what) {
    snprintf(g_err, sizeof(g_err), "%s: %s", what, cudaGetErrorString(e));
    return METIS_E_CUDA;
}
static int arg_fail(const char *what) {
    snprintf(g_err, sizeof(g_err), "%s", what);
    return METIS_E_ARG;
}
int fail_cuda(cudaError_t e, const char *what) { return cuda_fail(e, what); }
int fail_arg(const char *what) { return arg_fail(what); }

__device__ __forceinline__ void copy_bytes(uint8_t *dst, const void *src, uint32_t n, uint32_t tid, uint32_t nthr) {
    const uint8_t *s = static_cast<const uint8_t *>(src);
    for (uint32_t i = tid; i < n; i += nthr) dst[i] = s[i];
}

__global__ void pack_tables_kernel(MetisProblem p, BlobLayout l, uint8_t *blob) {
    const uint32_t tid = blockIdx.x * blockDim.x + threadIdx.x, nthr = gridDim.x * blockDim.x;
    const uint32_t nkey = (uint32_t)p.num_types * p.num_tp * p.num_bs;
    copy_bytes(blob + l.key, p.key_index, nkey * 2, tid, nthr);
    copy_bytes(blob + l.lc, p.layer_compute, (uint32_t)p.num_keys * p.lpad * 8, tid, nthr);
    copy_bytes(blob + l.mem, p.layer_memory, (uint32_t)p.num_keys * p.lpad * 8, tid, nthr);
    copy_bytes(blob + l.exec_full, p.exec_full, (uint32_t)p.num_keys * 8, tid, nthr);
    copy_bytes(blob + l.fb, p.fb_sync, (uint32_t)p.num_keys * 8, tid, nthr);
    copy_bytes(blob + l.norm, p.norm_lc, (uint32_t)p.norm_len * 8, tid, nthr);
    copy_bytes(blob + l.tmem, p.type_memory, (uint32_t)p.num_types * 8, tid, nthr);
    copy_bytes(blob + l.bwf, p.type_bw_first, (uint32_t)p.num_types * 8, tid, nthr);
    copy_bytes(blob + l.bwm, p.type_bw_min, (uint32_t)p.num_types * 8, tid, nthr);
    copy_bytes(blob + l.runt, p.ns_run_type, (uint32_t)p.num_node_sequences * p.num_types, tid, nthr);
    copy_bytes(blob + l.rune, p.ns_run_end, (uint32_t)p.num_node_sequences * p.num_types * 4, tid, nthr);
    copy_bytes(blob + l.q10e, p.ns_q10_end, (uint32_t)p.num_node_sequences * p.num_types * 4, tid, nthr);
    double *derived = reinterpret_cast<double *>(blob + l.derived);
    const DerivedLayout d = derived_layout(p);
    for (uint32_t i = tid; i < (uint32_t)d.total; i += nthr)
        derived[i] = derive_entry(p, d, p.norm_lc, p.exec_full, p.type_bw_first, (int)i);
}

__global__ void __launch_bounds__(128)
range_sums_kernel(MetisProblem p, BlobLayout l, uint8_t *blob) {
    const int L = p.num_layers;
    const long long i = (long long)blockIdx.x * blockDim.x + threadIdx.x;
    if (i >= (long long)range_sum_tables(p) * L) return;
    const int t = (int)(i / L), a = (int)(i % L);
    const double *row = range_sum_row(p, t, p.layer_memory, p.layer_compute, p.norm_lc);
    if (!row) return;
    const size_t n = (size_t)L + 1;
    fill_range_sums(row, L, a, reinterpret_cast<double *>(blob + l.rsum) + (size_t)t * n * n);
}

__device__ __forceinline__ uint32_t smem_u32(const void *p) {
    return static_cast<uint32_t>(__cvta_generic_to_shared(p));
}

__device__ __forceinline__ void stage_blob_tma(uint8_t *smem, const uint8_t *blob, uint32_t bytes, uint64_t *mbar) {
    const uint32_t bar = smem_u32(mbar);
    if (threadIdx.x == 0) {
        asm volatile("mbarrier.init.shared::cta.b64 [%0], 1;" ::"r"(bar) : "memory");
        asm volatile("fence.mbarrier_init.release.cluster;" ::: "memory");
    }
    __syncthreads();
    if (threadIdx.x == 0) {
        asm volatile("mbarrier.arrive.expect_tx.shared::cta.b64 _, [%0], %1;" ::"r"(bar), "r"(bytes) : "memory");
        constexpr uint32_t kChunk = 32768;
        for (uint32_t off = 0; off < bytes; off += kChunk) {
            const uint32_t n = (bytes - off < kChunk) ? bytes - off : kChunk;
            asm volatile(
                "cp.async.bulk.shared::cluster.global.mbarrier::complete_tx::bytes [%0], [%1], %2, [%3];"
                ::"r"(smem_u32(smem + off)), "l"(blob + off), "r"(n), "r"(bar)
                : "memory");
        }
    }
    uint32_t done = 0;
    while (!done) {
        asm volatile(
            "{\n\t.reg .pred p;\n\t"
            "mbarrier.try_wait.parity.shared::cta.b64 p, [%1], 0;\n\t"
            "selp.u32 %0, 1, 0, p;\n\t}"
            : "=r"(done)
            : "r"(bar)
            : "memory");
    }
}

__device__ __forceinline__ const Tables &block_tables(Tables &s_tables, const MetisProblem &p, const BlobLayout &lay,
                                                      const uint8_t *blob, uint8_t *smem, int use_smem, uint64_t *mbar) {
    if (threadIdx.x == 0) s_tables = make_tables(p, lay, use_smem ? smem : blob, blob);
    if (use_smem) stage_blob_tma(smem, blob, lay.total, mbar);
    else __syncthreads();
    return s_tables;
}

__device__ __forceinline__ void decode_task(const MetisPlanSpace &sp, uint64_t hdr, uint64_t geo, PlanDesc &pd) {
    pd.ordinal = (uint32_t)hdr;
    pd.geo = geo;
    pd.row = sp.rows + (geo & 0xFFFFFFFFULL);
    pd.S = (int)((geo >> 32) & 0xFF) + 1;
    pd.label = (int)((geo >> 40) & 0xFF) + 1;
    pd.ns = (int)((geo >> 48) & 0xFF);
    pd.batches = __ldg(&sp.batches[(geo >> 56) & 0xFF]);
}

__device__ __forceinline__ bool rec_less(double c0, uint32_t o0, uint32_t s0, double c1, uint32_t o1, uint32_t s1) {
    if (c0 < c1) return true;
    if (c0 > c1) return false;
    if (o0 != o1) return o0 < o1;
    return s0 < s1;
}

struct DeviceOut {
    MetisRecord *records;
    long long capacity;
    uint8_t *detail;
    int detail_stride;
    unsigned long long *counters;
    MetisRecord *block_best;
};

struct DeviceSink {
    const DeviceOut &o;
    unsigned int n_part, n_run, n_key;
    double best_cost;
    uint32_t best_ord, best_step, best_meta;
    bool leader;
    __device__ DeviceSink(const DeviceOut &out)
        : o(out), n_part(0), n_run(0), n_key(0), best_cost(INFINITY), best_ord(0xFFFFFFFFu), best_step(0xFFFFu),
          best_meta(0), leader(true) {}
    __device__ DeviceSink(const DeviceOut &out, double *) : DeviceSink(out) {}
#ifdef METIS_PROFILE_PHASES
    __device__ void phase(int id) { bulk_mark(0xFFFFFFFFu, id); }
#else
    __device__ void phase(int) {}
#endif
    __device__ void partition_call() { n_part += leader ? 1u : 0u; }
    __device__ void balancer_run() { n_run += leader ? 1u : 0u; }
    __device__ void keyerror() { n_key += leader ? 1u : 0u; }
    __device__ void fatal(uint32_t ordinal, int code, uint32_t aux) {
        if (!leader) return;
        const unsigned long long key = ((unsigned long long)ordinal << 32) | ((unsigned long long)(code & 0xFF) << 24) |
                                       (unsigned long long)(((aux >> 16) & 0xFF) << 16) | (aux & 0xFFFF);
        atomicMin(&o.counters[4], key);
    }
    __device__ void emit(const PlanDesc &pd, int step, int nrep, double cost, const uint8_t *tpc, const uint16_t *part) {
        emit_with(pd, step, nrep, cost, tpc, part, [](unsigned long long) {});
    }
    template <class Also>
    __device__ void emit_with(const PlanDesc &pd, int step, int nrep, double cost, const uint8_t *tpc,
                              const uint16_t *part, const Also &also) {
        if (!leader) return;
        const unsigned long long slot = atomicAdd(&o.counters[0], 1ULL);
        if ((long long)slot < o.capacity) {
            MetisRecord r;
            r.cost = cost; r.ordinal = pd.ordinal; r.step = (uint16_t)step;
            r.num_repartition = (uint8_t)nrep; r.num_stage = (uint8_t)pd.S;
            o.records[slot] = r;
            also(slot);
            if (o.detail) {
                uint8_t *d = o.detail + (size_t)slot * o.detail_stride;
                for (int s = 0; s < pd.S; ++s) { d[s] = (uint8_t)(pd.row[s] - tpc[s]); d[pd.S + s] = tpc[s]; }
                for (int s = 0; s <= pd.S; ++s) d[2 * pd.S + s] = (uint8_t)part[s];
            }
        }
        if (rec_less(cost, pd.ordinal, (uint32_t)step, best_cost, best_ord, best_step)) {
            best_cost = cost; best_ord = pd.ordinal; best_step = (uint32_t)step;
            best_meta = ((uint32_t)nrep << 8) | (uint32_t)pd.S;
        }
    }
};

struct HeadroomSink : DeviceSink {
    double *headroom;
    const double *state;
    __device__ HeadroomSink(const DeviceOut &out, double *h) : DeviceSink(out), headroom(h), state(nullptr) {}
    __device__ void emit(const PlanDesc &pd, int step, int nrep, double cost, const uint8_t *tpc, const uint16_t *part) {
        emit_with(pd, step, nrep, cost, tpc, part, [&](unsigned long long slot) {
            double m = state[0];
            for (int s = 1; s < pd.S; ++s)
                if (state[s] < m) m = state[s];
            headroom[slot] = m;
        });
    }
};

struct MissOut {
    MetisMiss *misses;
    long long capacity;
};

static_assert(METIS_MAX_STAGES * 30 + 1 < (1 << 14), "MetisMiss.key: call index may not fit in 14 bits");
template <class Base>
struct MissSink : Base {
    static constexpr bool kMisses = true;
    MissOut mo;
    int call;
    __device__ MissSink(const DeviceOut &out, double *h, const MissOut &m) : Base(out, h), mo(m), call(0) {}
    __device__ void miss(const PlanDesc &pd, int attempt, double deficit, int stage) {
        if (!this->leader) return;
        const unsigned long long slot = atomicAdd(&this->o.counters[5], 1ULL);
        if ((long long)slot < mo.capacity) {
            MetisMiss r;
            r.deficit = deficit; r.ordinal = pd.ordinal; r.key = (uint16_t)((call << 2) | attempt);
            r.stage = (uint8_t)stage; r.num_stage = (uint8_t)pd.S;
            mo.misses[slot] = r;
        }
    }
};

constexpr int kOutHeadroom = 1, kOutMisses = 2;
template <int OUT>
struct SinkOf {
    using Plain = typename std::conditional<(OUT & kOutHeadroom) != 0, HeadroomSink, DeviceSink>::type;
    using type = typename std::conditional<(OUT & kOutMisses) != 0, MissSink<Plain>, Plain>::type;
};
template <int OUT, class S = typename SinkOf<OUT>::type>
__device__ __forceinline__ S make_sink(const DeviceOut &out, double *headroom, const MissOut &m) {
    if constexpr ((OUT & kOutMisses) != 0) return S(out, headroom, m);
    else return S(out, headroom);
}

__device__ __forceinline__ void finish_block(const DeviceSink &sink, const DeviceOut &out, int slot) {
    __shared__ double s_cost[32];
    __shared__ uint32_t s_ord[32], s_step[32], s_meta[32];
    const unsigned full = 0xFFFFFFFFu;
    const unsigned np = __reduce_add_sync(full, sink.n_part);
    const unsigned nr = __reduce_add_sync(full, sink.n_run);
    const unsigned nk = __reduce_add_sync(full, sink.n_key);
    const int lane = threadIdx.x & 31, warp = threadIdx.x >> 5;
    if (lane == 0) {
        if (np) atomicAdd(&out.counters[1], (unsigned long long)np);
        if (nr) atomicAdd(&out.counters[2], (unsigned long long)nr);
        if (nk) atomicAdd(&out.counters[3], (unsigned long long)nk);
    }
    double c = sink.best_cost;
    uint32_t o = sink.best_ord, st = sink.best_step, mt = sink.best_meta;
    for (int d = 16; d > 0; d >>= 1) {
        const double c2 = __shfl_xor_sync(full, c, d);
        const uint32_t o2 = __shfl_xor_sync(full, o, d), s2 = __shfl_xor_sync(full, st, d),
                       m2 = __shfl_xor_sync(full, mt, d);
        if (rec_less(c2, o2, s2, c, o, st)) { c = c2; o = o2; st = s2; mt = m2; }
    }
    if (lane == 0) { s_cost[warp] = c; s_ord[warp] = o; s_step[warp] = st; s_meta[warp] = mt; }
    __syncthreads();
    if (threadIdx.x == 0) {
        const int nw = (blockDim.x + 31) >> 5;
        for (int wi = 1; wi < nw; ++wi)
            if (rec_less(s_cost[wi], s_ord[wi], s_step[wi], c, o, st)) { c = s_cost[wi]; o = s_ord[wi]; st = s_step[wi]; mt = s_meta[wi]; }
        MetisRecord r;
        r.cost = c; r.ordinal = o; r.step = (uint16_t)st; r.num_repartition = (uint8_t)(mt >> 8); r.num_stage = (uint8_t)mt;
        out.block_best[slot] = r;
    }
}

struct SearchLists {
    uint4 *a, *b;
    unsigned int *ctl;
    long long bulk_min;
    double *perf;
    unsigned int *src;
    unsigned int save_cap;
};
constexpr int kCtlHist = 16, kCtlCursor = 16 + 160;
constexpr int kCtlHist2 = 512, kCtlCursor2 = 512 + 160;
constexpr int kCtlHist3 = 832, kCtlCursor3 = 832 + 160;
constexpr unsigned kHintMax = 127;

__device__ __forceinline__ uint4 make_entry(uint32_t ordinal, uint32_t flags, uint64_t geo) {
    return make_uint4(ordinal, flags, (uint32_t)geo, (uint32_t)(geo >> 32));
}
__device__ __forceinline__ void decode_entry(const MetisPlanSpace &sp, const uint4 e, PlanDesc &pd) {
    decode_task(sp, (uint64_t)e.x, ((uint64_t)e.w << 32) | e.z, pd);
}

__global__ void __launch_bounds__(256)
het_admit_kernel(const __grid_constant__ MetisPlanSpace sp, const MetisShard sh, const long long slots,
                 const int gbs, const int max_bs, const int max_tp, const SearchLists ls) {
    const int lane = threadIdx.x & 31;
    const long long b0 = ((long long)blockIdx.x * blockDim.x + threadIdx.x) & ~31LL;
    if (b0 >= slots) return;
    const long long first = ((b0 / sh.tile) * sh.world + sh.rank) * sh.tile + (b0 % sh.tile);
    int hint = 0;
    if (lane == 0 && first < sp.num_plans) hint = find_block(sp, first);
    hint = __shfl_sync(0xFFFFFFFFu, hint, 0);
    PlanDesc pd;
    int halvings = 0;
    bool ok = b0 + lane < slots && decode_plan(sp, first + lane, pd, hint);
    if (ok) {
        const int bs_total = gbs / pd.batches;
        const int lb = 31 - __clz(bs_total > 0 ? bs_total : 1);
        const int ltp = 31 - __clz(max_tp > 0 ? max_tp : 1), lbs = 31 - __clz(max_bs > 0 ? max_bs : 1);
        if (bs_total <= 0) ok = false;
        for (int s = 0; ok && s < pd.S; ++s) {
            const int g = __ldg(&pd.row[s]);
            const int t = g > lb ? g - lb : 0;
            const int mbs = bs_total >> (g - t);
            if (mbs == 0 || mbs > max_bs || (1 << t) > max_tp) ok = false;
            else {
                const int lm = 31 - __clz(mbs);
                int room = g - t;
                room = min(room, min(ltp - t, lbs - lm));
                if (room > 0) halvings += room;
            }
        }
    }
    const unsigned full = 0xFFFFFFFFu;
    const unsigned m = __ballot_sync(full, ok);
    if (m == 0) return;
    const int leader = __ffs(m) - 1;
    unsigned int base = 0;
    if (lane == leader) base = atomicAdd(&ls.ctl[0], (unsigned int)__popc(m));
    base = __shfl_sync(full, base, leader);
    const int k = ok ? pd.S - 1 : -1;
    const unsigned peers = __match_any_sync(full, k);
    const unsigned key = (unsigned)halvings > kHintMax ? kHintMax : (unsigned)halvings;
    const unsigned peers3 = __match_any_sync(full, ok ? (int)key : -1);
    if (ok) {
        ls.a[base + __popc(m & ((1u << lane) - 1u))] = make_entry(pd.ordinal, key << 8, pd.geo);
        if (lane == __ffs(peers) - 1) atomicAdd(&ls.ctl[kCtlHist + k], (unsigned int)__popc(peers));
        if (lane == __ffs(peers3) - 1) atomicAdd(&ls.ctl[kCtlHist3 + key], (unsigned int)__popc(peers3));
    }
}

__global__ void __launch_bounds__(256)
het_scatter_kernel(const SearchLists ls) {
    __shared__ unsigned int s_base[160];
    const unsigned int n = ls.ctl[0];
    const bool bulk = (long long)n >= ls.bulk_min;
    const int hist = bulk ? kCtlHist : kCtlHist3, cursor = bulk ? kCtlCursor : kCtlCursor3;
    if (threadIdx.x == 0) {
        unsigned int acc = 0;
        for (int k = 127; k >= 0; --k) { s_base[k] = acc; acc += ls.ctl[hist + k]; }
    }
    __syncthreads();
    const long long span = (long long)gridDim.x * blockDim.x;
    const long long upto = (((long long)n + 31) / 32) * 32;
    for (long long pos = (long long)blockIdx.x * blockDim.x + threadIdx.x; pos < upto; pos += span) {
        const bool live = pos < (long long)n;
        uint4 e = make_uint4(0, 0, 0, 0);
        if (live) e = ls.a[pos];
        const int k = !live ? -1 : bulk ? (int)(e.w & 0xFF) : (int)((e.y >> 8) & 0x7F);
        const unsigned int peers = __match_any_sync(0xFFFFFFFFu, k);
        const int leader = __ffs(peers) - 1, me = threadIdx.x & 31;
        unsigned int at = 0;
        if (live && me == leader) at = atomicAdd(&ls.ctl[cursor + k], (unsigned int)__popc(peers));
        at = __shfl_sync(0xFFFFFFFFu, at, leader);
        if (live) ls.b[(long long)s_base[k] + at + __popc(peers & ((1u << me) - 1u))] = e;
    }
}

template <int MAXS, int MAXL, bool ONE, int OUT>
__global__ void __launch_bounds__(kThreads, (MAXS <= 64 ? METIS_MIN_BLOCKS : ONE ? METIS_MIN_BLOCKS_BIG_ONE : METIS_MIN_BLOCKS_BIG))
het_first_kernel(const __grid_constant__ MetisProblem p, const __grid_constant__ MetisPlanSpace sp,
                 const __grid_constant__ BlobLayout lay, const uint8_t *__restrict__ blob, const int use_smem,
                 const __grid_constant__ DeviceOut out, const SearchLists ls, const int best_slot, double *headroom,
                 const MissOut misses) {
    extern __shared__ __align__(128) uint8_t smem[];
    __shared__ uint64_t mbar;
    __shared__ Tables s_tables;
    auto sink = make_sink<OUT>(out, headroom, misses);
    const unsigned int n = ls.ctl[0];
    if ((long long)n >= ls.bulk_min) {
        const Tables &T = block_tables(s_tables, p, lay, blob, smem, use_smem, &mbar);
        Scratch<MAXS, MAXL> w;
        if constexpr ((OUT & kOutHeadroom) != 0) sink.state = w.mstate;
        const int lane = threadIdx.x & 31;
        for (;;) {
            unsigned int fetched = 0;
            if (lane == 0) fetched = atomicAdd(&ls.ctl[1], 1u);
            const long long b0 = 32LL * __shfl_sync(0xFFFFFFFFu, fetched, 0);
            if (b0 >= (long long)n) break;
            const long long pos = b0 + lane;
            PlanDesc pd;
            const bool has = pos < (long long)n;
            uint4 e = make_uint4(0, 0, 0, 0);
            if (has) { e = ls.b[pos]; decode_entry(sp, e, pd); }
            int hint = 0, start = 1;
            const bool cont = first_task<MAXS, MAXL, ONE, Lockstep>(T, w, sink, has, pd, hint, start);
            const unsigned m = __ballot_sync(0xFFFFFFFFu, cont);
            if (m) {
                const int leader = __ffs(m) - 1;
                unsigned int at = 0;
                if (lane == leader) at = atomicAdd(&ls.ctl[2], (unsigned int)__popc(m));
                at = __shfl_sync(0xFFFFFFFFu, at, leader);
                if (cont) {
                    const unsigned key = hint < 0 ? 0u : (hint > 127 ? 127u : (unsigned)hint);
                    const unsigned int c = at + __popc(m & ((1u << lane) - 1u));
                    if (start == 2) {
                        if (c < ls.save_cap) {
                            for (int s = 0; s < pd.S; ++s) ls.perf[(size_t)s * ls.save_cap + c] = w.perf[s];
                        } else start = 1;
                    }
                    e.y = 1u | ((unsigned)start << 1) | (key << 8);
                    ls.a[c] = e;
                    atomicAdd(&ls.ctl[kCtlHist2 + key], 1u);
                }
            }
        }
    }
    finish_block(sink, out, best_slot + blockIdx.x);
}

__global__ void __launch_bounds__(256)
het_order_kernel(const SearchLists ls) {
    __shared__ unsigned int s_base[128];
    if ((long long)ls.ctl[0] < ls.bulk_min) return;
    const unsigned int n = ls.ctl[2];
    if (threadIdx.x == 0) {
        unsigned int acc = 0;
        for (int k = 127; k >= 0; --k) { s_base[k] = acc; acc += ls.ctl[kCtlHist2 + k]; }
    }
    __syncthreads();
    const long long span = (long long)gridDim.x * blockDim.x;
    for (long long pos = (long long)blockIdx.x * blockDim.x + threadIdx.x; pos < (long long)n; pos += span) {
        const uint4 e = ls.a[pos];
        const unsigned key = (e.y >> 8) & 0x7Fu;
        const unsigned int to = s_base[key] + atomicAdd(&ls.ctl[kCtlCursor2 + key], 1u);
        ls.b[to] = e;
        ls.src[to] = (unsigned int)pos;
    }
}

template <int MAXS, int MAXL>
struct alignas(16) ChainScratch {
    Scratch<MAXS, MAXL> w;
    CoopMail mail;
};


template <int MAXS, int MAXL, bool ONE, int OUT>
__global__ void __launch_bounds__(512, 2)
het_chain_kernel(const __grid_constant__ MetisProblem p, const __grid_constant__ MetisPlanSpace sp,
                 const __grid_constant__ BlobLayout lay, const uint8_t *__restrict__ blob, const int use_smem,
                 const unsigned int scratch_off, const __grid_constant__ DeviceOut out, const SearchLists ls,
                 const int best_slot, double *headroom, const MissOut misses) {
    extern __shared__ __align__(128) uint8_t smem[];
    __shared__ uint64_t mbar;
    __shared__ Tables s_tables;
    WarpCoop::prof_init();
    const Tables &T = block_tables(s_tables, p, lay, blob, smem, use_smem, &mbar);
    auto sink = make_sink<OUT>(out, headroom, misses);
    const int lane = threadIdx.x & 31;
    sink.leader = lane == 0;
    ChainScratch<MAXS, MAXL> *cs = reinterpret_cast<ChainScratch<MAXS, MAXL> *>(smem + scratch_off) + (threadIdx.x >> 5);
    if constexpr ((OUT & kOutHeadroom) != 0) sink.state = cs->w.mstate;
    const unsigned int n_adm = ls.ctl[0];
    const bool bulk = (long long)n_adm >= ls.bulk_min;
    const uint4 *list = ls.b;
    const unsigned int n = bulk ? ls.ctl[2] : n_adm;
    ChainCoop lanes;
    CoopEvaluator<MAXS, MAXL, ChainCoop, ONE> ev(T, cs->w, cs->mail, lanes);
    for (;;) {
        unsigned int i = 0;
        if (lane == 0) i = atomicAdd(&ls.ctl[3], 1u);
        i = __shfl_sync(0xFFFFFFFFu, i, 0);
        if (i >= n) break;
        const uint4 e = __ldcg(&list[i]);
        PlanDesc pd;
        decode_entry(sp, e, pd);
        ev.x.mark(1);
        const int start = (e.y & 1u) ? (int)((e.y >> 1) & 3u) : 0;
        const double *perf = nullptr;
        if (start == 2) perf = ls.perf + __ldcg(&ls.src[i]);
        ev.run_chain(pd, sink, start, perf, (size_t)ls.save_cap);
        ev.x.mark(0);
    }
    ev.x.mark(25);
    while (WarpCoop::block_or(0)) {}
    ev.x.mark(31);
    sink.leader = true;
    if (lane != 0) { sink.n_part = sink.n_run = sink.n_key = 0; }
    finish_block(sink, out, best_slot + blockIdx.x);
}

__global__ void het_finalize_kernel(const MetisRecord *block_best, int nblocks, const unsigned long long *counters,
                                    const unsigned int *ctl, unsigned long long instantiation, MetisSearchSummary *summary) {
    __shared__ double s_cost[32];
    __shared__ uint32_t s_ord[32], s_step[32], s_meta[32];
    double c = INFINITY;
    uint32_t o = 0xFFFFFFFFu, st = 0xFFFFu, mt = 0;
    for (int i = threadIdx.x; i < nblocks; i += blockDim.x) {
        const MetisRecord r = block_best[i];
        if (rec_less(r.cost, r.ordinal, r.step, c, o, st)) {
            c = r.cost; o = r.ordinal; st = r.step; mt = ((uint32_t)r.num_repartition << 8) | r.num_stage;
        }
    }
    const unsigned full = 0xFFFFFFFFu;
    for (int d = 16; d > 0; d >>= 1) {
        const double c2 = __shfl_xor_sync(full, c, d);
        const uint32_t o2 = __shfl_xor_sync(full, o, d), s2 = __shfl_xor_sync(full, st, d),
                       m2 = __shfl_xor_sync(full, mt, d);
        if (rec_less(c2, o2, s2, c, o, st)) { c = c2; o = o2; st = s2; mt = m2; }
    }
    const int lane = threadIdx.x & 31, warp = threadIdx.x >> 5;
    if (lane == 0) { s_cost[warp] = c; s_ord[warp] = o; s_step[warp] = st; s_meta[warp] = mt; }
    __syncthreads();
    if (threadIdx.x == 0) {
        const int nw = (blockDim.x + 31) / 32;
        for (int wi = 1; wi < nw; ++wi)
            if (rec_less(s_cost[wi], s_ord[wi], s_step[wi], c, o, st)) { c = s_cost[wi]; o = s_ord[wi]; st = s_step[wi]; mt = s_meta[wi]; }
        MetisSearchSummary s;
        memset(&s, 0, sizeof(s));
        s.num_records = counters[0];
        s.num_partition_calls = counters[1];
        s.num_balancer_runs = counters[2];
        s.num_keyerror = counters[3];
        const unsigned long long fk = counters[4];
        if (fk == 0xFFFFFFFFFFFFFFFFULL) { s.fatal_ordinal = 0xFFFFFFFFFFFFFFFFULL; s.fatal_code = 0; s.fatal_aux = 0; }
        else { s.fatal_ordinal = fk >> 32; s.fatal_code = (uint32_t)((fk >> 24) & 0xFF); s.fatal_aux = (uint32_t)(fk & 0xFFFFFF); }
        s.best.cost = c; s.best.ordinal = o; s.best.step = (uint16_t)st;
        s.best.num_repartition = (uint8_t)(mt >> 8); s.best.num_stage = (uint8_t)mt;
        s.reserved[0] = ctl[0];
        s.reserved[1] = ctl[2];
        s.reserved[2] = instantiation;
        s.reserved[3] = counters[5];
        *summary = s;
    }
}

struct DetailSink {
    uint8_t *dst;
    int want_step;
    __device__ void phase(int) {}
    __device__ void partition_call() {}
    __device__ void balancer_run() {}
    __device__ void keyerror() {}
    __device__ void fatal(uint32_t, int, uint32_t) {}
    __device__ void emit(const PlanDesc &pd, int step, int, double, const uint8_t *tpc, const uint16_t *part) {
        if (step != want_step) return;
        for (int s = 0; s < pd.S; ++s) { dst[s] = (uint8_t)(pd.row[s] - tpc[s]); dst[pd.S + s] = tpc[s]; }
        for (int s = 0; s <= pd.S; ++s) dst[2 * pd.S + s] = (uint8_t)part[s];
    }
};

template <int MAXS, int MAXL>
__global__ void __launch_bounds__(kThreads)
het_detail_kernel(const __grid_constant__ MetisProblem p, const __grid_constant__ MetisPlanSpace sp,
                  const __grid_constant__ BlobLayout lay, const uint8_t *__restrict__ blob,
                  const MetisRecord *__restrict__ picks, long long n, uint8_t *detail, int stride) {
    const Tables T = make_tables(p, lay, blob);
    const long long i = (long long)blockIdx.x * kThreads + threadIdx.x;
    if (i >= n) return;
    PlanDesc pd;
    if (!decode_plan(sp, picks[i].ordinal, pd)) return;
    DetailSink sink{detail + (size_t)i * stride, (int)picks[i].step};
    Scratch<MAXS, MAXL> w;
    PlanEvaluator<MAXS, MAXL> ev(T, w);
    ev.run(pd, sink, (int)picks[i].step);
}

__global__ void __launch_bounds__(64)
het_trace_kernel(const __grid_constant__ MetisProblem p, const __grid_constant__ MetisPlanSpace sp,
                 const __grid_constant__ BlobLayout lay, const uint8_t *__restrict__ blob,
                 const uint32_t *__restrict__ ordinals, long long n, uint64_t *trace, int words) {
    const Tables T = make_tables(p, lay, blob);
    const long long i = (long long)blockIdx.x * blockDim.x + threadIdx.x;
    if (i >= n) return;
    TraceOut out(trace + (size_t)i * words, words);
    PlanDesc pd;
    if (decode_plan(sp, ordinals[i], pd)) {
        Scratch<kMaxS, kMaxL> w;
        TraceEvaluator<kMaxS, kMaxL> ev(T, w, out);
        ev.run_traced(pd);
    }
    out.finish();
}

__global__ void __launch_bounds__(kThreads)
het_breakdown_kernel(const __grid_constant__ MetisProblem p, const __grid_constant__ MetisPlanSpace sp,
                     const __grid_constant__ BlobLayout lay, const uint8_t *__restrict__ blob,
                     const MetisRecord *__restrict__ picks, long long n, MetisBreakdown *out, double *stage_out,
                     int stride) {
    const Tables T = make_tables(p, lay, blob);
    const long long i = (long long)blockIdx.x * kThreads + threadIdx.x;
    if (i >= n || (i > 0 && picks[i - 1].ordinal == picks[i].ordinal)) return;
    long long end = i + 1;
    while (end < n && picks[end].ordinal == picks[i].ordinal) ++end;
    Scratch<kMaxS, kMaxL> w;
    BreakdownEvaluator<kMaxS, kMaxL> ev(T, w, picks, i, end, out, stage_out, stride);
    for (long long k = i; k < end; ++k) ev.clear(k);
    PlanDesc pd;
    if (decode_plan(sp, picks[i].ordinal, pd)) ev.replay(pd);
}

__global__ void __launch_bounds__(kThreads)
homo_breakdown_kernel(const __grid_constant__ MetisProblem p, const __grid_constant__ BlobLayout lay,
                      const uint8_t *__restrict__ blob, int type_id, const int32_t *__restrict__ plans, long long n,
                      double *terms, double *stage_memory, int stride, int32_t *status) {
    const Tables T = make_tables(p, lay, blob);
    const long long i = (long long)blockIdx.x * kThreads + threadIdx.x;
    if (i >= n) return;
    status[i] = homo_breakdown(T, type_id, plans + i * 5, terms + i * 6, stage_memory + i * stride, stride);
}

__global__ void __launch_bounds__(kThreads)
homo_cost_kernel(const __grid_constant__ MetisProblem p, const __grid_constant__ BlobLayout lay,
                 const uint8_t *__restrict__ blob, int type_id, const int32_t *__restrict__ plans, long long n,
                 double *cost, int32_t *status) {
    const Tables T = make_tables(p, lay, blob);
    const long long i = (long long)blockIdx.x * kThreads + threadIdx.x;
    if (i >= n) return;
    const int32_t *q = plans + i * 5;
    double c = 0.0;
    int oom = 0;
    const int rc = homo_cost(T, type_id, q[0], q[1], q[2], q[3], q[4], c, oom);
    cost[i] = rc ? NAN : c;
    status[i] = rc ? 1 : (oom ? 2 : 0);
}

template <int MAXS, int MAXL>
__global__ void __launch_bounds__(kThreads)
layer_balance_kernel(const double *__restrict__ capa, const int32_t *__restrict__ num_stage, long long n, int stride,
                     const double *__restrict__ lc, const double *__restrict__ dlay, int norm_len, int num_layers,
                     uint16_t *partition) {
    const long long i = (long long)blockIdx.x * kThreads + threadIdx.x;
    if (i >= n) return;
    Tables T;
    memset(&T, 0, sizeof(T));
    T.p.num_layers = num_layers;
    T.p.norm_len = norm_len;
    T.norm_lc = lc;
    T.dlay = dlay;
    Scratch<MAXS, MAXL> w;
    const int S = num_stage[i];
    uint16_t *out = partition + i * (stride + 1);
    if (S < 1 || S > MAXS || num_layers > MAXL) { out[0] = 0xFFFF; return; }
    for (int s = 0; s < S; ++s) w.perf[s] = capa[i * stride + s];
    const int rc = balance_run<MAXS, MAXL>(T, S, w, Serial());
    if (rc) { out[0] = 0xFFFF; return; }
    for (int s = 0; s <= S; ++s) out[s] = w.part[s];
}

constexpr int kRowWarps = 8;
__global__ void __launch_bounds__(kRowWarps * 32)
het_rows_kernel(const MetisCompRec *__restrict__ recs, long long ncomp, const uint8_t *__restrict__ pool,
                uint8_t *__restrict__ rows) {
    __shared__ CompWalk s_walk[kRowWarps];
    __shared__ uint8_t s_pool[kRowWarps][METIS_MAX_PERMUTE_GROUPS + METIS_MAX_STAGES];
    const unsigned full = 0xFFFFFFFFu;
    const int lane = threadIdx.x & 31, wid = threadIdx.x >> 5;
    const long long c = (long long)blockIdx.x * kRowWarps + wid;
    if (c >= ncomp) return;
    const MetisCompRec rec = recs[c];
    const int stages = rec.stages, n = rec.num_groups;
    if (stages > METIS_MAX_STAGES || n > METIS_MAX_PERMUTE_GROUPS) return;
    for (int p = lane; p < n + stages; p += 32) s_pool[wid][p] = pool[rec.pool_offset + p];
    __syncwarp();
    CompWalk &cw = s_walk[wid];
    MetisCompRec local = rec;
    local.pool_offset = 0;
    if (lane == 0) {
        cw.init(local, s_pool[wid]);
        for (uint32_t skip = 0; skip < rec.first_row; ++skip) cw.advance();
    }
    uint8_t *dst = rows + rec.row_offset;
    for (uint32_t r = 0;;) {
        __syncwarp();
        int at = 0;
        for (int h = cw.head; h >= 0; h = cw.nxt[h]) {
            const int len = cw.len[h], off = cw.off[h];
            for (int b = lane; b < len; b += 32) dst[at + b] = cw.codes[off + b];
            at += len;
        }
        __syncwarp();
        if (++r >= rec.num_rows) break;
        int more = 0;
        if (lane == 0) more = cw.advance() ? 1 : 0;
        if (!__shfl_sync(full, more, 0)) break;
        dst += stages;
    }
}

__global__ void divide_by_seven_kernel(const double *lc, int n, double *out) {
    const int i = blockIdx.x * blockDim.x + threadIdx.x;
    if (i < n) out[i] = lc[i] / 7.0;
}

static int check_problem(const MetisProblem *p) {
    if (!p) return arg_fail("problem is NULL");
    if (p->num_types < 1 || p->num_types > METIS_MAX_TYPES) return arg_fail("num_types out of range");
    if (p->num_layers < 1 || p->num_layers > METIS_MAX_LAYERS || p->num_layers > 255)
        return arg_fail("num_layers out of range (1 .. 255)");
    if (p->lpad < p->num_layers) return arg_fail("lpad < num_layers");
    if (p->num_keys < 1 || p->num_tp < 1 || p->num_bs < 1 || p->norm_len < 1) return arg_fail("empty profile tables");
    if (p->devices_per_node < 1 || p->total_devices < 1 || p->q10_devices < 1) return arg_fail("empty cluster");
    return METIS_OK;
}

}

using namespace metis;

extern "C" {

const char *metis_last_error(void) { return g_err; }
int metis_abi_version(void) { return METIS_ABI_VERSION; }
#ifdef METIS_PROFILE_PHASES
int metis_debug_marks(long long *out32, int reset) {
    long long zero[64] = {0};
    if (out32) cudaMemcpyFromSymbol(out32, g_mark_acc, sizeof(zero));
    if (reset) cudaMemcpyToSymbol(g_mark_acc, zero, sizeof(zero));
    return 0;
}
int metis_debug_bulk_marks(long long *out32, int reset) {
    long long zero[32] = {0};
    if (out32) cudaMemcpyFromSymbol(out32, g_bulk_acc, sizeof(zero));
    if (reset) cudaMemcpyToSymbol(g_bulk_acc, zero, sizeof(zero));
    return 0;
}
#endif
void metis_set_profile_events(void *before_kernel, void *after_kernel) {
    g_ev_before = static_cast<cudaEvent_t>(before_kernel);
    g_ev_after = static_cast<cudaEvent_t>(after_kernel);
}

static int64_t shard_plan_slots(int64_t num_plans, const MetisShard *sh) {
    const int64_t tile = sh->tile, world = sh->world;
    const int64_t rounds = (num_plans + tile * world - 1) / (tile * world);
    return rounds * tile;
}

constexpr int64_t kFixedWs = 16384;
constexpr int64_t kMaxBlocks = 4096;

static int env_int(const char *name, int lo, int hi, int dflt) {
    const char *e = getenv(name);
    if (!e || !*e) return dflt;
    char *end = nullptr;
    const long v = strtol(e, &end, 10);
    if (end == e || *end != '\0' || v < lo || v > hi) return dflt;
    return (int)v;
}

static int64_t save_slots(int64_t cap) {
    const int forced = env_int("METIS_SAVE_SLOTS", 1, 1 << 20, 0);
    if (forced) return forced;
    return cap / 4 < 131072 ? (cap / 4 > 0 ? cap / 4 : 1) : 131072;
}

int64_t metis_het_workspace_bytes(const MetisProblem *problem, int64_t num_plans, int32_t max_stage) {
    if (check_problem(problem)) return METIS_E_ARG;
    if (num_plans < 0) return METIS_E_ARG;
    const BlobLayout lay = make_layout(*problem);
    const int64_t cap = (num_plans + 127) & ~(int64_t)127;
    const int64_t stages = max_stage < 1 ? 1 : (max_stage > METIS_MAX_STAGES ? METIS_MAX_STAGES : max_stage);
    return 256 + kFixedWs + (int64_t)lay.rsum + (int64_t)align16(lay.rsum_bytes) + kMaxBlocks * (int64_t)sizeof(MetisRecord) +
           2 * cap * (int64_t)sizeof(uint4) + cap * 4 + save_slots(cap) * stages * 8 + 1024;
}

struct Workspace {
    MetisSearchSummary *summary;
    unsigned long long *counters;
    unsigned int *ctl;
    uint8_t *blob;
    MetisRecord *block_best;
    uint8_t *lists;
};

static Workspace carve(void *ws, const BlobLayout &lay) {
    uint8_t *b = static_cast<uint8_t *>(ws);
    uintptr_t a = (reinterpret_cast<uintptr_t>(b) + 127) & ~(uintptr_t)127;
    b = reinterpret_cast<uint8_t *>(a);
    Workspace w;
    w.summary = reinterpret_cast<MetisSearchSummary *>(b);
    w.counters = reinterpret_cast<unsigned long long *>(b + 1024);
    w.ctl = reinterpret_cast<unsigned int *>(b + 2048);
    w.blob = b + kFixedWs;
    w.block_best = reinterpret_cast<MetisRecord *>(b + kFixedWs + lay.rsum + align16(lay.rsum_bytes));
    w.lists = reinterpret_cast<uint8_t *>(w.block_best + kMaxBlocks);
    return w;
}


}

template <int MAXS, int MAXL, bool ONE, int OUT>
static int launch_search(const MetisProblem &p_arg, const MetisPlanSpace &s_arg, const MetisShard &sh,
                         const BlobLayout &lay, const Workspace &ws, const DeviceOut &out, double *headroom,
                         const MissOut &misses, int64_t slots, cudaStream_t stream) {
    cudaError_t e;
    int dev = 0, sms = 0, smem_optin = 0;
    cudaGetDevice(&dev);
    cudaDeviceGetAttribute(&sms, cudaDevAttrMultiProcessorCount, dev);
    cudaDeviceGetAttribute(&smem_optin, cudaDevAttrMaxSharedMemoryPerBlockOptin, dev);
    if (sms < 1 || smem_optin < 48 * 1024) return cuda_fail(cudaErrorInvalidDevice, "device attributes");
    const int blob_max = env_int("METIS_SMEM_BLOB_MAX", 0, kSmemBlobMax, kSmemBlobMax);
    const unsigned int blob_pad = (lay.total + 127u) & ~127u;

    SearchLists ls;
    const int64_t cap = (slots + 127) & ~(int64_t)127;
    ls.a = reinterpret_cast<uint4 *>(ws.lists);
    ls.b = ls.a + cap;
    ls.ctl = ws.ctl;
    ls.src = reinterpret_cast<unsigned int *>(ls.b + cap);
    ls.perf = reinterpret_cast<double *>(ls.src + cap);
    ls.save_cap = (unsigned int)save_slots(cap);

    auto chain = het_chain_kernel<MAXS, MAXL, ONE, OUT>;
    const size_t per_warp = sizeof(ChainScratch<MAXS, MAXL>);
    int chain_smem_tables = (int)lay.total <= blob_max;
    int chain_threads = 0, chain_per_sm = 0;
    size_t chain_dyn = 0;
    unsigned int chain_off = 0;
    const int forced = env_int("METIS_CHAIN_THREADS", 32, 512, 0);
    for (int pass = 0; pass < 2 && chain_threads == 0; ++pass) {
        int best_warps = 0;
        for (int threads = 64; threads <= 512; threads *= 2) {
            if (forced && threads != ((forced + 31) & ~31)) continue;
            const unsigned int off = chain_smem_tables ? blob_pad : 0u;
            const size_t dyn = off + (size_t)(threads / 32) * per_warp;
            if (dyn > (size_t)smem_optin) continue;
            e = cudaFuncSetAttribute(chain, cudaFuncAttributeMaxDynamicSharedMemorySize, (int)dyn);
            if (e != cudaSuccess) { cudaGetLastError(); continue; }
            int per_sm = 0;
            e = cudaOccupancyMaxActiveBlocksPerMultiprocessor(&per_sm, chain, threads, dyn);
            if (e != cudaSuccess || per_sm < 1) { cudaGetLastError(); continue; }
            const int warps = per_sm * threads / 32;
            if (warps > best_warps) { best_warps = warps; chain_threads = threads; chain_per_sm = per_sm; chain_dyn = dyn; chain_off = off; }
        }
        if (chain_threads == 0) chain_smem_tables = 0;
    }
    if (chain_threads == 0) return arg_fail("chain kernel does not fit this device (shared memory)");
    e = cudaFuncSetAttribute(chain, cudaFuncAttributeMaxDynamicSharedMemorySize, (int)chain_dyn);
    if (e != cudaSuccess) return cuda_fail(e, "cudaFuncSetAttribute(chain)");
    int64_t chain_grid = (int64_t)sms * chain_per_sm;

    auto first = het_first_kernel<MAXS, MAXL, ONE, OUT>;
    int first_smem_tables = (int)lay.total <= blob_max && blob_pad <= (unsigned int)smem_optin;
    size_t first_dyn = first_smem_tables ? blob_pad : 0;
    e = cudaFuncSetAttribute(first, cudaFuncAttributeMaxDynamicSharedMemorySize, (int)first_dyn);
    if (e != cudaSuccess) { cudaGetLastError(); first_smem_tables = 0; first_dyn = 0; }
    int first_per_sm = 0;
    e = cudaOccupancyMaxActiveBlocksPerMultiprocessor(&first_per_sm, first, kThreads, first_dyn);
    if (e != cudaSuccess || first_per_sm < 1) return cuda_fail(e, "occupancy query (bulk round)");
    int64_t first_grid = (int64_t)sms * first_per_sm;
    if (first_grid + chain_grid > kMaxBlocks) return arg_fail("grid exceeds the per-block best table");

    ls.bulk_min = sh.reserved > 0 ? (long long)sh.reserved : 12LL * chain_grid * (chain_threads / 32);

    if (g_ev_before) cudaEventRecord(g_ev_before, stream);
    if (slots > 0) {
        const int64_t admit_blocks = (slots + 255) / 256;
        if (admit_blocks > 0x7FFFFFFFLL) return arg_fail("too many plans for one launch");
        het_admit_kernel<<<(unsigned)admit_blocks, 256, 0, stream>>>(s_arg, sh, (long long)slots, p_arg.gbs, p_arg.max_bs,
                                                                     p_arg.max_tp, ls);
        int64_t scatter_blocks = (slots + 255) / 256;
        if (scatter_blocks > 8LL * sms) scatter_blocks = 8LL * sms;
        het_scatter_kernel<<<(unsigned)scatter_blocks, 256, 0, stream>>>(ls);
        first<<<(unsigned)first_grid, kThreads, first_dyn, stream>>>(p_arg, s_arg, lay, ws.blob, first_smem_tables, out, ls, 0,
                                                                  headroom, misses);
        het_order_kernel<<<(unsigned)(2 * sms), 256, 0, stream>>>(ls);
        chain<<<(unsigned)chain_grid, chain_threads, chain_dyn, stream>>>(p_arg, s_arg, lay, ws.blob, chain_smem_tables,
                                                                         chain_off, out, ls, (int)first_grid, headroom,
                                                                         misses);
        e = cudaGetLastError();
        if (e != cudaSuccess) return cuda_fail(e, "search kernels");
    }
    if (g_ev_after) cudaEventRecord(g_ev_after, stream);
    g_ev_before = g_ev_after = nullptr;
    const unsigned long long instantiation = (unsigned long long)MAXS | (unsigned long long)MAXL << 16 |
                                             (unsigned long long)ONE << 32;
    het_finalize_kernel<<<1, 256, 0, stream>>>(ws.block_best, (int)(slots > 0 ? first_grid + chain_grid : 0), ws.counters,
                                               ws.ctl, instantiation, ws.summary);
    e = cudaGetLastError();
    if (e != cudaSuccess) return cuda_fail(e, "het_finalize_kernel");
    return METIS_OK;
}

template <int OUT>
static int launch_tier(const MetisProblem &p, const MetisPlanSpace &sp, const MetisShard &sh, const BlobLayout &lay,
                       const Workspace &ws, const DeviceOut &out, double *headroom, const MissOut &m, int64_t slots,
                       cudaStream_t stream) {
    const bool one = p.num_types == 1;
    if (sp.max_stage <= 64 && p.num_layers <= 128)
        return one ? launch_search<64, 128, true, OUT>(p, sp, sh, lay, ws, out, headroom, m, slots, stream)
                   : launch_search<64, 128, false, OUT>(p, sp, sh, lay, ws, out, headroom, m, slots, stream);
    if (sp.max_stage <= 96 && p.num_layers <= 128)
        return one ? launch_search<96, 128, true, OUT>(p, sp, sh, lay, ws, out, headroom, m, slots, stream)
                   : launch_search<96, 128, false, OUT>(p, sp, sh, lay, ws, out, headroom, m, slots, stream);
    return one ? launch_search<kMaxS, kMaxL, true, OUT>(p, sp, sh, lay, ws, out, headroom, m, slots, stream)
               : launch_search<kMaxS, kMaxL, false, OUT>(p, sp, sh, lay, ws, out, headroom, m, slots, stream);
}

extern "C" {

int metis_het_search(const MetisProblem *problem, const MetisPlanSpace *space, const MetisShard *shard,
                     MetisRecord *records, int64_t capacity, uint8_t *detail, int32_t detail_stride,
                     void *workspace, int64_t workspace_bytes, MetisSearchSummary *summary, void *stream_) {
    return metis_het_search_headroom(problem, space, shard, records, capacity, detail, detail_stride, nullptr, workspace,
                                     workspace_bytes, summary, stream_);
}

int metis_het_search_headroom(const MetisProblem *problem, const MetisPlanSpace *space, const MetisShard *shard,
                              MetisRecord *records, int64_t capacity, uint8_t *detail, int32_t detail_stride,
                              double *headroom, void *workspace, int64_t workspace_bytes, MetisSearchSummary *summary,
                              void *stream_) {
    return metis_het_search_outputs(problem, space, shard, records, capacity, detail, detail_stride, headroom, nullptr, 0,
                                    workspace, workspace_bytes, summary, stream_);
}

int metis_het_search_outputs(const MetisProblem *problem, const MetisPlanSpace *space, const MetisShard *shard,
                             MetisRecord *records, int64_t capacity, uint8_t *detail, int32_t detail_stride,
                             double *headroom, MetisMiss *misses, int64_t miss_capacity, void *workspace,
                             int64_t workspace_bytes, MetisSearchSummary *summary, void *stream_) {
    int rc = check_problem(problem);
    if (rc) return rc;
    if (!space || !shard || !workspace || !summary) return arg_fail("NULL argument");
    if (shard->world < 1 || shard->rank < 0 || shard->rank >= shard->world || shard->tile < 32 || shard->tile % 32)
        return arg_fail("bad shard (tile must be a positive multiple of 32)");
    if (space->num_plans > 0xFFFFFFF0LL) return arg_fail("more than 2^32 plans");
    if (space->max_stage < 1 || space->max_stage > METIS_MAX_STAGES) return arg_fail("max_stage out of range (METIS_MAX_STAGES)");
    if (space->num_div < 1 || space->num_div > 256) return arg_fail("more than 256 divisors of gbs");
    if (problem->num_node_sequences < 1 || problem->num_node_sequences > 256)
        return arg_fail("more than 256 node sequences (geometry word)");
    if (space->rows_bytes < 0 || space->rows_bytes > 0xFFFFFFFFLL) return arg_fail("row tables must be smaller than 4 GiB (geometry word)");
    if (detail && detail_stride < 3 * space->max_stage + 1) return arg_fail("detail_stride too small (3 * max_stage + 1)");
    if (capacity < 0 || (capacity > 0 && !records)) return arg_fail("records/capacity mismatch");
    if (headroom && !records) return arg_fail("headroom without records");
    if (miss_capacity < 0 || (miss_capacity > 0 && !misses)) return arg_fail("misses/miss_capacity mismatch");
    cudaStream_t stream = static_cast<cudaStream_t>(stream_);
    const BlobLayout lay = make_layout(*problem);
    const int64_t slots = shard_plan_slots(space->num_plans, shard);
    const int64_t need = metis_het_workspace_bytes(problem, slots, space->max_stage);
    if (workspace_bytes < need) { snprintf(g_err, sizeof(g_err), "workspace too small: need %lld", (long long)need); return METIS_E_CAPACITY; }
    const Workspace ws = carve(workspace, lay);

    cudaError_t e;
    e = cudaMemsetAsync(ws.counters, 0, kFixedWs - 1024, stream);
    if (e != cudaSuccess) return cuda_fail(e, "memset counters");
    e = cudaMemsetAsync(ws.counters + 4, 0xFF, sizeof(unsigned long long), stream);
    if (e != cudaSuccess) return cuda_fail(e, "memset fatal key");
    pack_tables_kernel<<<8, 256, 0, stream>>>(*problem, lay, ws.blob);
    {
        const long long nthr = (long long)range_sum_tables(*problem) * problem->num_layers;
        range_sums_kernel<<<(unsigned)((nthr + 127) / 128), 128, 0, stream>>>(*problem, lay, ws.blob);
    }
    e = cudaGetLastError();
    if (e != cudaSuccess) return cuda_fail(e, "pack_tables_kernel");

    DeviceOut out;
    out.records = records; out.capacity = capacity; out.detail = detail; out.detail_stride = detail_stride;
    out.counters = ws.counters; out.block_best = ws.block_best;
    MissOut mo;
    mo.misses = misses; mo.capacity = misses ? miss_capacity : 0;
    const int outs = (headroom ? kOutHeadroom : 0) | (misses ? kOutMisses : 0);
    switch (outs) {
    case 0: rc = launch_tier<0>(*problem, *space, *shard, lay, ws, out, nullptr, mo, slots, stream); break;
    case kOutHeadroom: rc = launch_tier<kOutHeadroom>(*problem, *space, *shard, lay, ws, out, headroom, mo, slots, stream); break;
    case kOutMisses: rc = launch_tier<kOutMisses>(*problem, *space, *shard, lay, ws, out, nullptr, mo, slots, stream); break;
    default: rc = launch_tier<kOutHeadroom | kOutMisses>(*problem, *space, *shard, lay, ws, out, headroom, mo, slots, stream);
    }
    if (rc) return rc;
    e = cudaMemcpyAsync(summary, ws.summary, sizeof(MetisSearchSummary), cudaMemcpyDeviceToHost, stream);
    if (e != cudaSuccess) return cuda_fail(e, "copy summary");
    return METIS_OK;
}

int metis_het_detail(const MetisProblem *problem, const MetisPlanSpace *space, const MetisRecord *picks, int64_t n,
                     uint8_t *detail, int32_t detail_stride, void *workspace, int64_t workspace_bytes, void *stream_) {
    int rc = check_problem(problem);
    if (rc) return rc;
    if (!space || !picks || !detail || !workspace) return arg_fail("NULL argument");
    if (detail_stride < 3 * space->max_stage + 1) return arg_fail("detail_stride too small (3 * max_stage + 1)");
    cudaStream_t stream = static_cast<cudaStream_t>(stream_);
    const BlobLayout lay = make_layout(*problem);
    if (workspace_bytes < 256 + kFixedWs + (int64_t)align16(lay.total)) return METIS_E_CAPACITY;
    const Workspace ws = carve(workspace, lay);
    pack_tables_kernel<<<8, 256, 0, stream>>>(*problem, lay, ws.blob);
    if (n > 0) {
        const unsigned nb = (unsigned)((n + kThreads - 1) / kThreads);
        het_detail_kernel<kMaxS, kMaxL><<<nb, kThreads, 0, stream>>>(*problem, *space, lay, ws.blob, picks, n, detail,
                                                                     detail_stride);
    }
    cudaError_t e = cudaGetLastError();
    if (e != cudaSuccess) return cuda_fail(e, "het_detail_kernel");
    return METIS_OK;
}

}

int metis::stage_replay_tables(const MetisProblem *problem, void *workspace, int64_t workspace_bytes, cudaStream_t stream,
                               BlobLayout &lay, const uint8_t *&blob) {
    int rc = check_problem(problem);
    if (rc) return rc;
    if (!workspace) return arg_fail("NULL argument");
    lay = make_layout(*problem);
    if (workspace_bytes < 256 + kFixedWs + (int64_t)align16(lay.total)) return METIS_E_CAPACITY;
    const Workspace ws = carve(workspace, lay);
    pack_tables_kernel<<<8, 256, 0, stream>>>(*problem, lay, ws.blob);
    blob = ws.blob;
    return METIS_OK;
}

extern "C" {

int metis_het_trace(const MetisProblem *problem, const MetisPlanSpace *space, const uint32_t *ordinals, int64_t n,
                    uint64_t *trace, int32_t words_per_plan, void *workspace, int64_t workspace_bytes, void *stream_) {
    int rc = check_problem(problem);
    if (rc) return rc;
    if (!space || !ordinals || !trace || !workspace) return arg_fail("NULL argument");
    if (words_per_plan < 64) return arg_fail("words_per_plan too small");
    cudaStream_t stream = static_cast<cudaStream_t>(stream_);
    const BlobLayout lay = make_layout(*problem);
    if (workspace_bytes < 256 + kFixedWs + (int64_t)align16(lay.total)) return METIS_E_CAPACITY;
    const Workspace ws = carve(workspace, lay);
    pack_tables_kernel<<<8, 256, 0, stream>>>(*problem, lay, ws.blob);
    if (n > 0) {
        const unsigned nb = (unsigned)((n + 63) / 64);
        het_trace_kernel<<<nb, 64, 0, stream>>>(*problem, *space, lay, ws.blob, ordinals, n, trace, words_per_plan);
    }
    cudaError_t e = cudaGetLastError();
    if (e != cudaSuccess) return cuda_fail(e, "het_trace_kernel");
    return METIS_OK;
}

int metis_het_breakdown(const MetisProblem *problem, const MetisPlanSpace *space, const MetisRecord *picks, int64_t n,
                        MetisBreakdown *out, double *stage_out, int32_t stage_stride, void *workspace,
                        int64_t workspace_bytes, void *stream_) {
    int rc = check_problem(problem);
    if (rc) return rc;
    if (!space || (n > 0 && (!picks || !out)) || !workspace) return arg_fail("NULL argument");
    if (n < 0) return arg_fail("negative number of picks");
    if (stage_out && (stage_stride < 1 || stage_stride > METIS_MAX_STAGES)) return arg_fail("stage_stride out of range");
    cudaStream_t stream = static_cast<cudaStream_t>(stream_);
    const BlobLayout lay = make_layout(*problem);
    if (workspace_bytes < 256 + kFixedWs + (int64_t)align16(lay.total)) return METIS_E_CAPACITY;
    const Workspace ws = carve(workspace, lay);
    pack_tables_kernel<<<8, 256, 0, stream>>>(*problem, lay, ws.blob);
    if (n > 0) {
        const unsigned nb = (unsigned)((n + kThreads - 1) / kThreads);
        het_breakdown_kernel<<<nb, kThreads, 0, stream>>>(*problem, *space, lay, ws.blob, picks, n, out, stage_out,
                                                          stage_stride);
    }
    cudaError_t e = cudaGetLastError();
    if (e != cudaSuccess) return cuda_fail(e, "het_breakdown_kernel");
    return METIS_OK;
}

int metis_homo_breakdown(const MetisProblem *problem, int32_t type_id, const int32_t *plans, int64_t n, double *terms,
                         double *stage_memory, int32_t stage_stride, int32_t *status, void *workspace,
                         int64_t workspace_bytes, void *stream_) {
    int rc = check_problem(problem);
    if (rc) return rc;
    if (!plans || !terms || !stage_memory || !status || !workspace) return arg_fail("NULL argument");
    if (type_id < 0 || type_id >= problem->num_types) return arg_fail("type_id out of range");
    if (stage_stride < 1) return arg_fail("stage_stride out of range");
    cudaStream_t stream = static_cast<cudaStream_t>(stream_);
    const BlobLayout lay = make_layout(*problem);
    if (workspace_bytes < 256 + kFixedWs + (int64_t)align16(lay.total)) return METIS_E_CAPACITY;
    const Workspace ws = carve(workspace, lay);
    pack_tables_kernel<<<8, 256, 0, stream>>>(*problem, lay, ws.blob);
    if (n > 0) {
        const unsigned nb = (unsigned)((n + kThreads - 1) / kThreads);
        homo_breakdown_kernel<<<nb, kThreads, 0, stream>>>(*problem, lay, ws.blob, type_id, plans, n, terms, stage_memory,
                                                           stage_stride, status);
    }
    cudaError_t e = cudaGetLastError();
    if (e != cudaSuccess) return cuda_fail(e, "homo_breakdown_kernel");
    return METIS_OK;
}

int metis_generate_rows(const MetisCompRec *recs, int64_t num_comps, const uint8_t *pool, uint8_t *rows, void *stream_) {
    if (num_comps < 0 || (num_comps > 0 && (!recs || !pool || !rows))) return arg_fail("NULL argument");
    if (num_comps > 0) {
        const int64_t nb = (num_comps + kRowWarps - 1) / kRowWarps;
        if (nb > 0x7FFFFFFFLL) return arg_fail("too many compositions for one launch");
        het_rows_kernel<<<(unsigned)nb, kRowWarps * 32, 0, static_cast<cudaStream_t>(stream_)>>>(recs, (long long)num_comps, pool, rows);
    }
    cudaError_t e = cudaGetLastError();
    if (e != cudaSuccess) return cuda_fail(e, "het_rows_kernel");
    return METIS_OK;
}

int metis_homo_cost(const MetisProblem *problem, int32_t type_id, const int32_t *plans, int64_t n, double *cost,
                    int32_t *status, void *workspace, int64_t workspace_bytes, void *stream_) {
    int rc = check_problem(problem);
    if (rc) return rc;
    if (!plans || !cost || !status || !workspace) return arg_fail("NULL argument");
    if (type_id < 0 || type_id >= problem->num_types) return arg_fail("type_id out of range");
    cudaStream_t stream = static_cast<cudaStream_t>(stream_);
    const BlobLayout lay = make_layout(*problem);
    if (workspace_bytes < 256 + kFixedWs + (int64_t)align16(lay.total)) return METIS_E_CAPACITY;
    const Workspace ws = carve(workspace, lay);
    pack_tables_kernel<<<8, 256, 0, stream>>>(*problem, lay, ws.blob);
    if (n > 0) {
        const unsigned nb = (unsigned)((n + kThreads - 1) / kThreads);
        homo_cost_kernel<<<nb, kThreads, 0, stream>>>(*problem, lay, ws.blob, type_id, plans, n, cost, status);
    }
    cudaError_t e = cudaGetLastError();
    if (e != cudaSuccess) return cuda_fail(e, "homo_cost_kernel");
    return METIS_OK;
}

int metis_layer_balance(const double *capa, const int32_t *num_stage, int64_t n, int32_t stride, const double *lc,
                        int32_t norm_len, int32_t num_layers, uint16_t *partition, void *workspace,
                        int64_t workspace_bytes, void *stream_) {
    if (!capa || !num_stage || !lc || !partition || !workspace) return arg_fail("NULL argument");
    if (stride < 1 || stride > METIS_MAX_STAGES) return arg_fail("stride out of range");
    if (num_layers < 1 || num_layers > METIS_MAX_LAYERS || norm_len < 1) return arg_fail("layers out of range");
    if (workspace_bytes < (int64_t)norm_len * 8 + 256) return METIS_E_CAPACITY;
    cudaStream_t stream = static_cast<cudaStream_t>(stream_);
    double *dlay = reinterpret_cast<double *>((reinterpret_cast<uintptr_t>(workspace) + 127) & ~(uintptr_t)127);
    divide_by_seven_kernel<<<(norm_len + 127) / 128, 128, 0, stream>>>(lc, norm_len, dlay);
    if (n > 0) {
        const unsigned nb = (unsigned)((n + kThreads - 1) / kThreads);
        layer_balance_kernel<kMaxS, kMaxL><<<nb, kThreads, 0, stream>>>(capa, num_stage, n, stride, lc, dlay, norm_len,
                                                                        num_layers, partition);
    }
    cudaError_t e = cudaGetLastError();
    if (e != cudaSuccess) return cuda_fail(e, "layer_balance_kernel");
    return METIS_OK;
}

}
```

Before: 215.7 million.

## Access shared-memory lookup tables through 32-bit shared addresses instead of generic pointers

Templates the table struct on an address space so that, when the blob is staged in shared memory, every table is held as a 32-bit shared-window address and read with explicit ld.shared instructions instead of generic 64-bit loads. The evaluator, coop and search code paths are templated on the table type, and new kernel instantiations are selected at launch depending on whether the tables fit in shared memory. The specialised path is enabled only for the ONE (single device type) case. The aim is to cut generic-address conversion and register pressure in the hot lookup loops, at the cost of more template instantiations, longer compile times and larger code.

```diff
diff --git a/metis_b200/csrc/metis_blob.cuh b/metis_b200/csrc/metis_blob.cuh
--- a/metis_b200/csrc/metis_blob.cuh
+++ b/metis_b200/csrc/metis_blob.cuh
@@ -39,25 +39,31 @@
     return l;
 }
 
+template <class Space>
+__device__ __forceinline__ TablesOf<Space> bind_tables(const MetisProblem &p, const BlobLayout &l,
+                                                       typename Space::template ptr<uint8_t> base, const uint8_t *gblob) {
+    TablesOf<Space> T;
+    T.p = p;
+    T.rsum = gblob ? reinterpret_cast<const double *>(gblob + l.rsum) : nullptr;
+    T.key_index = tab_cast<int16_t>(base + l.key);
+    T.lc = tab_cast<double>(base + l.lc);
+    T.mem = tab_cast<double>(base + l.mem);
+    T.exec_full = tab_cast<double>(base + l.exec_full);
+    T.fb_sync = tab_cast<double>(base + l.fb);
+    T.norm_lc = tab_cast<double>(base + l.norm);
+    bind_derived(T, tab_cast<double>(base + l.derived));
+    T.type_memory = tab_cast<double>(base + l.tmem);
+    T.bw_first = tab_cast<double>(base + l.bwf);
+    T.bw_min = tab_cast<double>(base + l.bwm);
+    T.run_type = base + l.runt;
+    T.run_end = tab_cast<int32_t>(base + l.rune);
+    T.q10_end = tab_cast<int32_t>(base + l.q10e);
+    return T;
+}
+
 __device__ __forceinline__ Tables make_tables(const MetisProblem &p, const BlobLayout &l, const uint8_t *base,
                                               const uint8_t *gblob = nullptr) {
-    Tables T;
-    T.p = p;
-    T.rsum = gblob ? reinterpret_cast<const double *>(gblob + l.rsum) : nullptr;
-    T.key_index = reinterpret_cast<const int16_t *>(base + l.key);
-    T.lc = reinterpret_cast<const double *>(base + l.lc);
-    T.mem = reinterpret_cast<const double *>(base + l.mem);
-    T.exec_full = reinterpret_cast<const double *>(base + l.exec_full);
-    T.fb_sync = reinterpret_cast<const double *>(base + l.fb);
-    T.norm_lc = reinterpret_cast<const double *>(base + l.norm);
-    bind_derived(T, reinterpret_cast<const double *>(base + l.derived));
-    T.type_memory = reinterpret_cast<const double *>(base + l.tmem);
-    T.bw_first = reinterpret_cast<const double *>(base + l.bwf);
-    T.bw_min = reinterpret_cast<const double *>(base + l.bwm);
-    T.run_type = base + l.runt;
-    T.run_end = reinterpret_cast<const int32_t *>(base + l.rune);
-    T.q10_end = reinterpret_cast<const int32_t *>(base + l.q10e);
-    return T;
+    return bind_tables<GenericSpace>(p, l, base, gblob);
 }
 
 __device__ __forceinline__ int find_block(const MetisPlanSpace &sp, int64_t ordinal) {
diff --git a/metis_b200/csrc/metis_coop.cuh b/metis_b200/csrc/metis_coop.cuh
--- a/metis_b200/csrc/metis_coop.cuh
+++ b/metis_b200/csrc/metis_coop.cuh
@@ -67,10 +67,11 @@
     bool top_skip;
 };
 
-template <int MAXS, int MAXL>
-MB_HD_NOINLINE FillState seq_forward(const Tables &T, int S, Scratch<MAXS, MAXL> &w) {
+template <int MAXS, int MAXL, class TT>
+MB_HD_NOINLINE FillState seq_forward(const TT &T, int S, Scratch<MAXS, MAXL> &w) {
+    assume_shared_tables(T);
     const int L = T.p.num_layers;
-    const double *dlay = T.dlay;
+    const auto dlay = T.dlay;
     const int N = kH * L;
     const int lim = (N - 1 - kH) > 0 ? (N - 1 - kH) : 0;
     const int last = S - 1;
@@ -120,10 +121,11 @@
     return st;
 }
 
-template <int MAXS, int MAXL>
-MB_HD_NOINLINE int seq_backward(const Tables &T, int S, Scratch<MAXS, MAXL> &w, int k) {
+template <int MAXS, int MAXL, class TT>
+MB_HD_NOINLINE int seq_backward(const TT &T, int S, Scratch<MAXS, MAXL> &w, int k) {
+    assume_shared_tables(T);
     const int L = T.p.num_layers;
-    const double *dlay = T.dlay;
+    const auto dlay = T.dlay;
     const int N = kH * L;
     const int last = S - 1;
     double c = w.capa[last];
@@ -164,9 +166,10 @@
     return m;
 }
 
-template <int MAXS, int MAXL>
-MB_HD_NOINLINE int seq_skipped(const Tables &T, int S, Scratch<MAXS, MAXL> &w) {
-    const double *dlay = T.dlay;
+template <int MAXS, int MAXL, class TT>
+MB_HD_NOINLINE int seq_skipped(const TT &T, int S, Scratch<MAXS, MAXL> &w) {
+    assume_shared_tables(T);
+    const auto dlay = T.dlay;
     const int last = S - 1;
     int start = 0;
 #pragma unroll 1
@@ -264,33 +267,33 @@
 #endif
 }
 
-template <class X>
-MB_HD int psub_lookup(const X &x, const double *P, const uint16_t *IX, double scale, int N, int lo, double t, double &p) {
+template <class X, class PT, class IT>
+MB_HD int psub_lookup(const X &x, PT P, IT IX, double scale, int N, int lo, double t, double &p) {
     int i = IX[bucket_of(t * scale)];
     if (i < lo) i = lo;
-    const double *q = P + i;
+    const auto q = P + i;
     const double pm = q[-1], p0 = q[0], p1 = q[1];
     if ((pm < t || i == lo) && p1 >= t) {
         const bool up = !(p0 >= t);
         p = up ? p1 : p0;
         return up ? i + 1 : i;
     }
-    i = psub_search(x, P, N, i, lo, t);
+    i = psub_search(x, tab_generic(P), N, i, lo, t);
     p = P[i];
     return i;
 }
 
-template <int MAXS, int MAXL, class X, bool ONE = false>
-struct CoopEvaluator : PlanEvaluator<MAXS, MAXL, SerialUniform, ONE> {
-    using Base = PlanEvaluator<MAXS, MAXL, SerialUniform, ONE>;
+template <int MAXS, int MAXL, class X, bool ONE = false, class TT = Tables>
+struct CoopEvaluator : PlanEvaluator<MAXS, MAXL, SerialUniform, ONE, TT> {
+    using Base = PlanEvaluator<MAXS, MAXL, SerialUniform, ONE, TT>;
     using Base::T; using Base::w; using Base::pd; using Base::bs_total; using Base::nbad; using Base::aux;
     X x;
     CoopMail &mail;
 
-    MB_HD CoopEvaluator(const Tables &t, Scratch<MAXS, MAXL> &s, CoopMail &mb, const X &lanes)
+    MB_HD CoopEvaluator(const TT &t, Scratch<MAXS, MAXL> &s, CoopMail &mb, const X &lanes)
         : Base(t, s), x(lanes), mail(mb) {}
 
-    MB_HD void shared_scratch() const { X::assume_shared(&w); X::assume_shared(&mail); }
+    MB_HD void shared_scratch() const { X::assume_shared(&w); X::assume_shared(&mail); assume_shared_tables(T); }
 
     MB_HD void begin_coop(const PlanDesc &plan) {
         shared_scratch();
@@ -396,12 +399,12 @@
         if (S < 4 || T.p.norm_len < L) { x.note(kPathSeqForward); return false; }
         const int N = kH * L;
         const int lim = (N - 1 - kH) > 0 ? (N - 1 - kH) : 0;
-        const double *dsub = T.dsub;
-        const double *P = T.psub;
+        const auto dsub = T.dsub;
+        const auto P = T.psub;
         int a = 0, first_open = -1;
         const double scale = T.pidx[0];
         if (scale > 0.0) {
-            const uint16_t *IX = reinterpret_cast<const uint16_t *>(T.pidx + 1);
+            const auto IX = tab_cast<uint16_t>(T.pidx + 1);
             const double plim = P[lim];
             double pa = P[0];
             int s = 0;
@@ -431,8 +434,8 @@
                     const double t = w.perf[s] + P[a];
                     int i0 = a + span - 14;
                     if (i0 < a + 1) i0 = a + 1;
-                    int i = x.first_ge_window(P, N, i0, a + 1, t);
-                    if (i < 0) { x.note(kPathFirstGe); i = x.first_ge(P, N, t); }
+                    int i = x.first_ge_window(tab_generic(P), N, i0, a + 1, t);
+                    if (i < 0) { x.note(kPathFirstGe); i = x.first_ge(tab_generic(P), N, t); }
                     b = i - 1 > a ? i - 1 : a;
                     if (b >= lim) b = lim; else closed = true;
                     span = b - a;
@@ -476,7 +479,7 @@
     MB_HD int fill_coop() {
         shared_scratch();
         const int S = pd.S, last = S - 1;
-        const double *dlay = T.dlay;
+        const auto dlay = T.dlay;
         x.sync();
         const bool fwd = forward_coop();
         x.sync();
@@ -584,7 +587,7 @@
         const int S = pd.S;
         const int L = T.p.num_layers;
         if (T.p.norm_len < L) return METIS_FATAL_INDEX;
-        const double *lc = T.norm_lc;
+        const auto lc = T.norm_lc;
         const int last = S - 1;
         x.sync();
         METIS_PAR(x, s, S) { w.capa[s] = w.perf[s]; w.got[s] = 0; }
diff --git a/metis_b200/csrc/metis_eval.cuh b/metis_b200/csrc/metis_eval.cuh
--- a/metis_b200/csrc/metis_eval.cuh
+++ b/metis_b200/csrc/metis_eval.cuh
@@ -20,29 +20,72 @@
 constexpr double kMemCoef = 5.0;
 constexpr uint8_t kDropped = 0xFF;
 
-struct Tables {
+struct GenericSpace {
+    template <class V> using ptr = const V *;
+};
+template <class U, class V> MB_HD const U *tab_cast(const V *p) { return reinterpret_cast<const U *>(p); }
+template <class V> MB_HD const V *tab_generic(const V *p) { return p; }
+#if defined(__CUDACC__)
+__device__ __forceinline__ void lds(uint32_t a, double &v) { asm("ld.shared.f64 %0, [%1];" : "=d"(v) : "r"(a)); }
+__device__ __forceinline__ void lds(uint32_t a, int32_t &v) { asm("ld.shared.s32 %0, [%1];" : "=r"(v) : "r"(a)); }
+__device__ __forceinline__ void lds(uint32_t a, int16_t &v) { asm("ld.shared.s16 %0, [%1];" : "=h"(v) : "r"(a)); }
+__device__ __forceinline__ void lds(uint32_t a, uint16_t &v) { asm("ld.shared.u16 %0, [%1];" : "=h"(v) : "r"(a)); }
+__device__ __forceinline__ void lds(uint32_t a, uint8_t &v) {
+    uint32_t r;
+    asm("ld.shared.u8 %0, [%1];" : "=r"(r) : "r"(a));
+    v = (uint8_t)r;
+}
+template <class V>
+struct SmemTab {
+    uint32_t addr;
+    __device__ __forceinline__ V operator[](int i) const {
+        V v;
+        lds(addr + (uint32_t)i * (uint32_t)sizeof(V), v);
+        return v;
+    }
+    template <class I>
+    __device__ __forceinline__ SmemTab operator+(I i) const { return SmemTab{addr + (uint32_t)i * (uint32_t)sizeof(V)}; }
+};
+struct SharedSpace {
+    template <class V> using ptr = SmemTab<V>;
+};
+template <class U, class V> __device__ __forceinline__ SmemTab<U> tab_cast(SmemTab<V> p) { return SmemTab<U>{p.addr}; }
+template <class V> __device__ __forceinline__ const V *tab_generic(SmemTab<V> p) {
+    return static_cast<const V *>(__cvta_shared_to_generic(p.addr));
+}
+#endif
+
+template <class Space>
+struct TablesOf {
+    template <class V> using ptr = typename Space::template ptr<V>;
     MetisProblem p;
-    const int16_t *key_index;
-    const double *lc;
-    const double *mem;
-    const double *exec_full;
-    const double *fb_sync;
-    const double *norm_lc;
-    const double *type_memory, *bw_first, *bw_min;
-    const uint8_t *run_type;
-    const int32_t *run_end;
-    const int32_t *q10_end;
-    const double *dlay;
-    const double *inv_exec;
-    const double *ratio;
-    const double *dpk;
-    const double *pp_hidden;
-    const double *pp_vocab;
-    const double *psub;
-    const double *dsub;
-    const double *pidx;
+    ptr<int16_t> key_index;
+    ptr<double> lc;
+    ptr<double> mem;
+    ptr<double> exec_full;
+    ptr<double> fb_sync;
+    ptr<double> norm_lc;
+    ptr<double> type_memory, bw_first, bw_min;
+    ptr<uint8_t> run_type;
+    ptr<int32_t> run_end;
+    ptr<int32_t> q10_end;
+    ptr<double> dlay;
+    ptr<double> inv_exec;
+    ptr<double> ratio;
+    ptr<double> dpk;
+    ptr<double> pp_hidden;
+    ptr<double> pp_vocab;
+    ptr<double> psub;
+    ptr<double> dsub;
+    ptr<double> pidx;
     const double *rsum;
 };
+using Tables = TablesOf<GenericSpace>;
+
+template <class TT> MB_HD void assume_shared_tables(const TT &) {}
+#if defined(__CUDACC__)
+__device__ __forceinline__ void assume_shared_tables(const TablesOf<SharedSpace> &T) { __builtin_assume(__isShared(&T)); }
+#endif
 
 constexpr int kDpk = 16;
 
@@ -131,7 +174,8 @@
     return ((double)((int64_t)mbs * p.sequence_length * p.vocab_size) / (double)(1 << tpc)) / bw;
 }
 
-MB_HD void bind_derived(Tables &T, const double *base) {
+template <class TT, class B>
+MB_HD void bind_derived(TT &T, B base) {
     const DerivedLayout d = derived_layout(T.p);
     T.dlay = base + d.dlay;
     T.inv_exec = base + d.inv_exec;
@@ -296,8 +340,8 @@
 }
 
 enum RangeTable { kRangeMem = 0, kRangeLc = 1, kRangeNorm = 2 };
-template <class X>
-MB_HD double range_sum(const Tables &T, int family, int key, const double *row, int a, int b) {
+template <class X, class TT, class R>
+MB_HD double range_sum(const TT &T, int family, int key, R row, int a, int b) {
     if (a >= b) return 0.0;
     if (T.rsum && b <= T.p.num_layers) {
         const int n = T.p.num_layers + 1;
@@ -308,7 +352,7 @@
         return T.rsum[((size_t)t * n + b) * n + a];
 #endif
     }
-    return sum_range<X>(row, a, b);
+    return sum_range<X>(tab_generic(row), a, b);
 }
 
 struct PySum {
@@ -339,27 +383,30 @@
     return d;
 }
 
-MB_HD int type_of_rank(const Tables &T, int ns, int rank) {
+template <class TT>
+MB_HD int type_of_rank(const TT &T, int ns, int rank) {
     const int nt = T.p.num_types;
-    const int32_t *end = T.run_end + ns * nt;
-    const uint8_t *typ = T.run_type + ns * nt;
+    const auto end = T.run_end + ns * nt;
+    const auto typ = T.run_type + ns * nt;
 #pragma unroll 1
     for (int k = 0; k < nt; ++k)
         if (rank < end[k]) return typ[k];
     return typ[nt - 1];
 }
 
-MB_HD int type_of_q10(const Tables &T, int ns, int idx) {
+template <class TT>
+MB_HD int type_of_q10(const TT &T, int ns, int idx) {
     const int nt = T.p.num_types;
-    const int32_t *end = T.q10_end + ns * nt;
-    const uint8_t *typ = T.run_type + ns * nt;
+    const auto end = T.q10_end + ns * nt;
+    const auto typ = T.run_type + ns * nt;
 #pragma unroll 1
     for (int k = 0; k < nt; ++k)
         if (idx < end[k]) return typ[k];
     return typ[nt - 1];
 }
 
-MB_HD int key_of(const Tables &T, int type, int tpc, int bs) {
+template <class TT>
+MB_HD int key_of(const TT &T, int type, int tpc, int bs) {
     if (tpc >= T.p.num_tp || bs < 1 || bs > T.p.num_bs) return -1;
     return T.key_index[(type * T.p.num_tp + tpc) * T.p.num_bs + (bs - 1)];
 }
@@ -447,12 +494,13 @@
     return (int)kDropped;
 }
 
-template <int MAXS, int MAXL, class X>
-MB_HD int balance_run(const Tables &T, int S, Scratch<MAXS, MAXL> &w, const X &x) {
+template <int MAXS, int MAXL, class X, class TT>
+MB_HD int balance_run(const TT &T, int S, Scratch<MAXS, MAXL> &w, const X &x) {
+    assume_shared_tables(T);
     const int L = T.p.num_layers;
     if (T.p.norm_len < L) return METIS_FATAL_INDEX;
-    const double *dlay = T.dlay;
-    const double *lc = T.norm_lc;
+    const auto dlay = T.dlay;
+    const auto lc = T.norm_lc;
     const int N = kH * L;
     const int lim = (N - 1 - kH) > 0 ? (N - 1 - kH) : 0;
     const int last = S - 1;
@@ -726,8 +774,10 @@
     int plus[METIS_MAX_TYPES];
 };
 
-MB_HD_NOINLINE int partition_data(const Tables &T, int ns, int rank_lo, int count, int dp, int tpc, int bs,
+template <class TT>
+MB_HD_NOINLINE int partition_data(const TT &T, int ns, int rank_lo, int count, int dp, int tpc, int bs,
                                   HSplit &out, uint32_t &aux, bool q10 = false) {
+    assume_shared_tables(T);
     const int gsz = count / dp;
     double perf[METIS_MAX_TYPES];
     PySum total;
@@ -822,9 +872,9 @@
     return (int)(code & 0xFF);
 }
 
-template <int MAXS, int MAXL, class X = Serial, bool ONE = false>
+template <int MAXS, int MAXL, class X = Serial, bool ONE = false, class TT = Tables>
 struct PlanEvaluator {
-    const Tables &T;
+    const TT &T;
     Scratch<MAXS, MAXL> &w;
     X x;
     PlanDesc pd;
@@ -833,7 +883,7 @@
     uint32_t aux;
     TraceTap *tap;
 
-    MB_HD PlanEvaluator(const Tables &t, Scratch<MAXS, MAXL> &s, const X &lanes = X())
+    MB_HD PlanEvaluator(const TT &t, Scratch<MAXS, MAXL> &s, const X &lanes = X())
         : T(t), w(s), x(lanes), bs_total(0), nbad(0), aux(0), tap(nullptr) {}
 
     MB_HD int group(int s) const { return 1 << w.gcode[s]; }
@@ -845,6 +895,7 @@
     }
 
     MB_HD int begin(const PlanDesc &plan) {
+        assume_shared_tables(T);
         pd = plan;
         if (pd.S > MAXS || T.p.num_layers > MAXL) return -1;
         bs_total = T.p.gbs / pd.batches;
@@ -895,8 +946,8 @@
     MB_HD double memory_capacity(int a, int b) const {
         const int nt = T.p.num_types;
         if (ONE || nt == 1) return T.type_memory[0] * (double)(b - a);
-        const int32_t *end = T.run_end + pd.ns * nt;
-        const uint8_t *typ = T.run_type + pd.ns * nt;
+        const auto end = T.run_end + pd.ns * nt;
+        const auto typ = T.run_type + pd.ns * nt;
         PySum acc;
         int lo = 0;
 #pragma unroll (X::kUniform ? 1 : 0)
@@ -924,6 +975,7 @@
     }
 
     MB_HD_NOINLINE int hetero_performance(int a, int b, int dp, int tpc, double &p) {
+        assume_shared_tables(T);
         HSplit hs;
         int rc = partition_data(T, pd.ns, a, b - a, dp, tpc, bs_total, hs, aux);
         if (rc) return rc;
@@ -1055,6 +1107,7 @@
 
 
     MB_HD int compute_performance() {
+        assume_shared_tables(T);
         PySum total;
         int rc = 0;
 #pragma unroll (X::kUniform ? 1 : 0)
@@ -1075,6 +1128,7 @@
     }
 
     MB_HD_NOINLINE int hetero_memory_demand(int s, int type0, double &demand) {
+        assume_shared_tables(T);
         const int la = w.part[s], lb = w.part[s + 1], tpc = w.tpc[s];
         HSplit hs;
         const int rc = partition_data(T, pd.ns, 0, T.p.q10_devices, dp_of(s), tpc, bs_total, hs, aux, true);
@@ -1097,6 +1151,7 @@
     }
 
     MB_HD_NOINLINE int memory_demand_own_type(int s, double &demand) {
+        assume_shared_tables(T);
         const int la = w.part[s], lb = w.part[s + 1], tpc = w.tpc[s], g = w.gcode[s];
         const int a = rank_start(s), b = a + (1 << g);
         const int ta = type_of_rank(T, pd.ns, a), tb = type_of_rank(T, pd.ns, b - 1);
@@ -1134,6 +1189,7 @@
     }
 
     MB_HD_NOINLINE int adjust_performance() {
+        assume_shared_tables(T);
         const int S = pd.S;
         double need = 0.;
         PySum avail_sum;
@@ -1179,6 +1235,7 @@
     }
     template <class Sink>
     MB_HD int memory_phase(int attempt, Sink &sink) {
+        assume_shared_tables(T);
         const int S = pd.S;
         bool oom = false;
         int rc = 0;
@@ -1214,6 +1271,7 @@
 
     template <class Sink>
     MB_HD_NOINLINE int partition_layer(Sink &sink) {
+        assume_shared_tables(T);
 #pragma unroll (X::kUniform ? 1 : 0)
         for (int attempt = 1; attempt <= 3; ++attempt) {
             sink.balancer_run();
@@ -1231,8 +1289,8 @@
         if (n0 == n1) return T.bw_first[type_of_q10(T, pd.ns, n0 * per)];
         double slow = INFINITY;
         const int nt = T.p.num_types;
-        const int32_t *end = T.q10_end + pd.ns * nt;
-        const uint8_t *typ = T.run_type + pd.ns * nt;
+        const auto end = T.q10_end + pd.ns * nt;
+        const auto typ = T.run_type + pd.ns * nt;
         int lo = 0;
 #pragma unroll (X::kUniform ? 1 : 0)
         for (int k = 0; k < nt; ++k) {
@@ -1270,6 +1328,7 @@
     }
 
     MB_HD_NOINLINE int hetero_exec_cost(int a, int b, int dp, int tpc, int la, int lb, double &len) {
+        assume_shared_tables(T);
         HSplit hs;
         uint32_t dummy;
         if (partition_data(T, pd.ns, a, b - a, dp, tpc, bs_total, hs, dummy)) return 1;
@@ -1298,8 +1357,8 @@
 
     MB_HD int fb_sync_cost(int a, int b, int tpc, int mbs, double &out) const {
         const int nt = T.p.num_types;
-        const int32_t *end = T.run_end + pd.ns * nt;
-        const uint8_t *typ = T.run_type + pd.ns * nt;
+        const auto end = T.run_end + pd.ns * nt;
+        const auto typ = T.run_type + pd.ns * nt;
         double mx = -INFINITY;
         int lo = 0;
 #pragma unroll (X::kUniform ? 1 : 0)
@@ -1319,6 +1378,7 @@
     }
 
     MB_HD int get_cost(double &cost_out) {
+        assume_shared_tables(T);
         const bool one_type = ONE || T.p.num_types == 1;
         const int nstage = pd.label < pd.S ? pd.label : pd.S;
         if (T.p.q10_devices < T.p.total_devices && rank_start(nstage) > T.p.q10_devices) return 1;
@@ -1392,10 +1452,11 @@
     }
 };
 
-template <int MAXS, int MAXL, bool ONE, class X = Serial, class Sink>
-MB_HD bool first_task(const Tables &T, Scratch<MAXS, MAXL> &w, Sink &sink, bool has, const PlanDesc &plan, int &chain_hint,
+template <int MAXS, int MAXL, bool ONE, class X = Serial, class Sink, class TT>
+MB_HD bool first_task(const TT &T, Scratch<MAXS, MAXL> &w, Sink &sink, bool has, const PlanDesc &plan, int &chain_hint,
                       int &resume) {
-    PlanEvaluator<MAXS, MAXL, X, ONE> ev(T, w);
+    assume_shared_tables(T);
+    PlanEvaluator<MAXS, MAXL, X, ONE, TT> ev(T, w);
     bool cont = false;
     sink.phase(1);
     if (has) {
diff --git a/metis_b200/csrc/metis_search.cu b/metis_b200/csrc/metis_search.cu
--- a/metis_b200/csrc/metis_search.cu
+++ b/metis_b200/csrc/metis_search.cu
@@ -121,9 +121,18 @@
     }
 }
 
-__device__ __forceinline__ const Tables &block_tables(Tables &s_tables, const MetisProblem &p, const BlobLayout &lay,
-                                                      const uint8_t *blob, uint8_t *smem, int use_smem, uint64_t *mbar) {
-    if (threadIdx.x == 0) s_tables = make_tables(p, lay, use_smem ? smem : blob, blob);
+template <bool SMEM>
+using SearchTables = TablesOf<typename std::conditional<SMEM, SharedSpace, GenericSpace>::type>;
+
+template <bool SMEM>
+__device__ __forceinline__ const SearchTables<SMEM> &block_tables(SearchTables<SMEM> &s_tables, const MetisProblem &p,
+                                                                  const BlobLayout &lay, const uint8_t *blob,
+                                                                  uint8_t *smem, int use_smem, uint64_t *mbar) {
+    if constexpr (SMEM) {
+        if (threadIdx.x == 0) s_tables = bind_tables<SharedSpace>(p, lay, SmemTab<uint8_t>{smem_u32(smem)}, blob);
+    } else {
+        if (threadIdx.x == 0) s_tables = make_tables(p, lay, use_smem ? smem : blob, blob);
+    }
     if (use_smem) stage_blob_tma(smem, blob, lay.total, mbar);
     else __syncthreads();
     return s_tables;
@@ -385,7 +394,7 @@
     }
 }
 
-template <int MAXS, int MAXL, bool ONE, int OUT>
+template <int MAXS, int MAXL, bool ONE, int OUT, bool SMEM>
 __global__ void __launch_bounds__(kThreads, (MAXS <= 64 ? METIS_MIN_BLOCKS : ONE ? METIS_MIN_BLOCKS_BIG_ONE : METIS_MIN_BLOCKS_BIG))
 het_first_kernel(const __grid_constant__ MetisProblem p, const __grid_constant__ MetisPlanSpace sp,
                  const __grid_constant__ BlobLayout lay, const uint8_t *__restrict__ blob, const int use_smem,
@@ -393,11 +402,11 @@
                  const MissOut misses) {
     extern __shared__ __align__(128) uint8_t smem[];
     __shared__ uint64_t mbar;
-    __shared__ Tables s_tables;
+    __shared__ SearchTables<SMEM> s_tables;
     auto sink = make_sink<OUT>(out, headroom, misses);
     const unsigned int n = ls.ctl[0];
     if ((long long)n >= ls.bulk_min) {
-        const Tables &T = block_tables(s_tables, p, lay, blob, smem, use_smem, &mbar);
+        const auto &T = block_tables<SMEM>(s_tables, p, lay, blob, smem, use_smem, &mbar);
         Scratch<MAXS, MAXL> w;
         if constexpr ((OUT & kOutHeadroom) != 0) sink.state = w.mstate;
         const int lane = threadIdx.x & 31;
@@ -464,7 +473,7 @@
 };
 
 
-template <int MAXS, int MAXL, bool ONE, int OUT>
+template <int MAXS, int MAXL, bool ONE, int OUT, bool SMEM>
 __global__ void __launch_bounds__(512, 2)
 het_chain_kernel(const __grid_constant__ MetisProblem p, const __grid_constant__ MetisPlanSpace sp,
                  const __grid_constant__ BlobLayout lay, const uint8_t *__restrict__ blob, const int use_smem,
@@ -472,9 +481,9 @@
                  const int best_slot, double *headroom, const MissOut misses) {
     extern __shared__ __align__(128) uint8_t smem[];
     __shared__ uint64_t mbar;
-    __shared__ Tables s_tables;
+    __shared__ SearchTables<SMEM> s_tables;
     WarpCoop::prof_init();
-    const Tables &T = block_tables(s_tables, p, lay, blob, smem, use_smem, &mbar);
+    const auto &T = block_tables<SMEM>(s_tables, p, lay, blob, smem, use_smem, &mbar);
     auto sink = make_sink<OUT>(out, headroom, misses);
     const int lane = threadIdx.x & 31;
     sink.leader = lane == 0;
@@ -485,7 +494,7 @@
     const uint4 *list = ls.b;
     const unsigned int n = bulk ? ls.ctl[2] : n_adm;
     ChainCoop lanes;
-    CoopEvaluator<MAXS, MAXL, ChainCoop, ONE> ev(T, cs->w, cs->mail, lanes);
+    CoopEvaluator<MAXS, MAXL, ChainCoop, ONE, SearchTables<SMEM>> ev(T, cs->w, cs->mail, lanes);
     for (;;) {
         unsigned int i = 0;
         if (lane == 0) i = atomicAdd(&ls.ctl[3], 1u);
@@ -821,6 +830,7 @@
     cudaDeviceGetAttribute(&smem_optin, cudaDevAttrMaxSharedMemoryPerBlockOptin, dev);
     if (sms < 1 || smem_optin < 48 * 1024) return cuda_fail(cudaErrorInvalidDevice, "device attributes");
     const int blob_max = env_int("METIS_SMEM_BLOB_MAX", 0, kSmemBlobMax, kSmemBlobMax);
+    constexpr bool SHARED = ONE;
     const unsigned int blob_pad = (lay.total + 127u) & ~127u;
 
     SearchLists ls;
@@ -832,7 +842,9 @@
     ls.perf = reinterpret_cast<double *>(ls.src + cap);
     ls.save_cap = (unsigned int)save_slots(cap);
 
-    auto chain = het_chain_kernel<MAXS, MAXL, ONE, OUT>;
+    auto chain_kernel = [](int smem_tables) {
+        return smem_tables ? het_chain_kernel<MAXS, MAXL, ONE, OUT, SHARED> : het_chain_kernel<MAXS, MAXL, ONE, OUT, false>;
+    };
     const size_t per_warp = sizeof(ChainScratch<MAXS, MAXL>);
     int chain_smem_tables = (int)lay.total <= blob_max;
     int chain_threads = 0, chain_per_sm = 0;
@@ -840,6 +852,7 @@
     unsigned int chain_off = 0;
     const int forced = env_int("METIS_CHAIN_THREADS", 32, 512, 0);
     for (int pass = 0; pass < 2 && chain_threads == 0; ++pass) {
+        const auto chain = chain_kernel(chain_smem_tables);
         int best_warps = 0;
         for (int threads = 64; threads <= 512; threads *= 2) {
             if (forced && threads != ((forced + 31) & ~31)) continue;
@@ -857,15 +870,24 @@
         if (chain_threads == 0) chain_smem_tables = 0;
     }
     if (chain_threads == 0) return arg_fail("chain kernel does not fit this device (shared memory)");
+    const auto chain = chain_kernel(chain_smem_tables);
     e = cudaFuncSetAttribute(chain, cudaFuncAttributeMaxDynamicSharedMemorySize, (int)chain_dyn);
     if (e != cudaSuccess) return cuda_fail(e, "cudaFuncSetAttribute(chain)");
     int64_t chain_grid = (int64_t)sms * chain_per_sm;
 
-    auto first = het_first_kernel<MAXS, MAXL, ONE, OUT>;
+    auto first = het_first_kernel<MAXS, MAXL, ONE, OUT, SHARED>;
     int first_smem_tables = (int)lay.total <= blob_max && blob_pad <= (unsigned int)smem_optin;
-    size_t first_dyn = first_smem_tables ? blob_pad : 0;
-    e = cudaFuncSetAttribute(first, cudaFuncAttributeMaxDynamicSharedMemorySize, (int)first_dyn);
-    if (e != cudaSuccess) { cudaGetLastError(); first_smem_tables = 0; first_dyn = 0; }
+    size_t first_dyn = blob_pad;
+    if (first_smem_tables) {
+        e = cudaFuncSetAttribute(first, cudaFuncAttributeMaxDynamicSharedMemorySize, (int)first_dyn);
+        if (e != cudaSuccess) { cudaGetLastError(); first_smem_tables = 0; }
+    }
+    if (!first_smem_tables) {
+        first = het_first_kernel<MAXS, MAXL, ONE, OUT, false>;
+        first_dyn = 0;
+        e = cudaFuncSetAttribute(first, cudaFuncAttributeMaxDynamicSharedMemorySize, 0);
+        if (e != cudaSuccess) cudaGetLastError();
+    }
     int first_per_sm = 0;
     e = cudaOccupancyMaxActiveBlocksPerMultiprocessor(&first_per_sm, first, kThreads, first_dyn);
     if (e != cudaSuccess || first_per_sm < 1) return cuda_fail(e, "occupancy query (bulk round)");
```

After: 224.5 million, median of 6. +4.1%, better.
